# unilight/jatts

Measured on AMD Instinct MI355X. Metric: audio samples/sec (22.05 kHz) + RTF, FastSpeech2+HiFi-GAN, higher is better.
Workload: dtype f32 (emulated: 3 exact bf16 terms per operand, 7 MFMA products, f32 accumulate; attention / norms / duration predictor exact f32); 1 GPU; FastSpeech2(JSUT conformer 4+4, adim 384)+HiFi-GAN v1 22k, 64 utts x 128 phonemes x 6 frames per GPU; hop=256, parallelism=dp1 (utterance sharding, int16 PCM all-gather)

## Files before the change

### include/jatts_hip.h

```cpp
#ifndef JATTS_HIP_H_
#define JATTS_HIP_H_

#include <stdint.h>

#ifdef __cplusplus
extern "C" {
#endif

#define JATTS_ABI_VERSION 7

#define JATTS_F32 0
#define JATTS_F16 1
#define JATTS_F32S 2
#define JATTS_F32E 3
#define JATTS_F32E6 4

#define JATTS_ACT_NONE 0
#define JATTS_ACT_RELU 1
#define JATTS_ACT_TANH 2
#define JATTS_ACT_SWISH 3
#define JATTS_ACT_MISH 4
#define JATTS_ACT_SNAKEBETA 5

#define JATTS_PAD_ZERO 0
#define JATTS_PAD_REFLECT 1

#define JATTS_PRE_NONE 0
#define JATTS_PRE_LRELU 1

#define JATTS_OK 0
#define JATTS_ERR_ARG (-1)
#define JATTS_ERR_HIP (-2)
#define JATTS_ERR_UNSUPPORTED (-3)

int jatts_abi_version(void);
const char* jatts_last_error(void);
int jatts_device_info(char* buf, int buflen);

typedef struct jatts_ragged {
  const int32_t* cu_rows;
  int32_t n_seq;
  int32_t max_len;
  int32_t len_mul;
  int32_t total_rows;
  const int32_t* host_lens;
} jatts_ragged;

typedef struct jatts_conv_desc {
  jatts_ragged rg;
  int32_t dtype;
  int32_t n_in;
  const void* x[3];
  int32_t ldx;
  float in_scale;
  int32_t pre_act;
  float pre_slope;
  const void* w;
  int32_t c_in;
  int32_t n_out;
  int32_t k_w;
  int32_t dil;
  int32_t pad;
  const float* bias;
  int32_t act;
  float alpha;
  const float* resid;
  int32_t ldr;
  void* y;
  int32_t ldy;
  int32_t y_is_f32;
  int32_t y_transposed;
  const int32_t* y_seq_col0;
  int32_t pad_mode;
  int32_t variant;
  const float* w_inv;
  const float* act_a;
  const float* act_b;
  int32_t n_split;
  int32_t ldy2;
  void* y2;
  const int32_t* y2_seq_col0;
  int32_t w_layout;
} jatts_conv_desc;

int jatts_conv1d(const jatts_conv_desc* d, void* stream);

int64_t jatts_conv_weight_index(int32_t n, int32_t tap, int32_t c, int32_t n_pad, int32_t c_in);

typedef struct jatts_resunit_desc {
  jatts_ragged rg;
  int32_t dtype;
  int32_t channels;
  int32_t k_w;
  int32_t dil;
  float slope;
  const void* x;
  void* y;
  const void* w1;
  const float* b1;
  const void* w2;
  const float* b2;
  const void* add0;
  const void* add1;
  float out_scale;
  const float* ws1;
  const float* ws2;
  int32_t w_layout;
  int32_t variant;
} jatts_resunit_desc;

int jatts_hifigan_resunit(const jatts_resunit_desc* d, void* stream);

int jatts_resunit_variant(const jatts_resunit_desc* d);

int jatts_resunit_single_conv(int32_t dtype, int32_t w_layout);

int64_t jatts_unit_weight_index_k32(int32_t n, int32_t tap, int32_t c, int32_t channels);

typedef struct jatts_resblock_desc {
  jatts_ragged rg;
  int32_t dtype;
  int32_t channels;
  int32_t k_w;
  int32_t n_units;
  int32_t dil[3];
  float slope;
  const void* x;
  void* y;
  const void* w1[3];
  const float* b1[3];
  const void* w2[3];
  const float* b2[3];
  const void* add0;
  const void* add1;
  float out_scale;
  const float* ws1[3];
  const float* ws2[3];
} jatts_resblock_desc;

int jatts_hifigan_resblock(const jatts_resblock_desc* d, void* stream);

int jatts_masked_loss(const jatts_ragged* rg, const float* a, int32_t lda, const float* b, int32_t ldb, int32_t dim,
                      const int32_t* valid_len, int32_t kind, float log_offset, double scale, float* out, double* workspace,
                      void* stream);
int jatts_conv1d_wgrad(const jatts_ragged* rg, const float* x, int32_t ldx, const float* dy, int32_t ldy, int32_t c_in,
                       int32_t n_out, int32_t k_w, int32_t dil, int32_t pad, float* dw, float* db, float* workspace, void* stream);
int jatts_pack_conv_weight(const float* w, int32_t n_out, int32_t c_in, int32_t k_w, int32_t c_mult, int32_t mode, int32_t dtype,
                           void* out, void* stream);
int jatts_pack_conv_weight_split(const float* w, int32_t n_out, int32_t c_in, int32_t k_w, int32_t c_mult, int32_t mode, void* out, float* inv,
                                 void* stream);
int jatts_pack_conv_weight_bf16x3(const float* w, int32_t n_out, int32_t c_in, int32_t k_w, int32_t c_mult, int32_t dgrad, void* out, void* stream);
int jatts_conv1d_wgrad_emul(const jatts_ragged* rg, const float* x, int32_t ldx, const float* dy, int32_t ldy, int32_t c_in, int32_t n_out, int32_t k_w,
                            int32_t dil, int32_t pad, int32_t dtype, float* dw, float* db, float* workspace, void* stream);
int jatts_col_sum(const float* x, int32_t ld, int64_t rows, int32_t dim, float* out, void* stream);

int jatts_layernorm_bwd(const float* x, int32_t ldx, const float* dy, int32_t lddy, const float* gamma, int64_t rows, int32_t dim,
                        float eps, float* dx, int32_t lddx, float* dgamma, float* dbeta, void* stream);
int jatts_act_fwd(int32_t mode, const float* x, float* y, int64_t n, void* stream);
int jatts_act_bwd(int32_t mode, const float* x, const float* dy, float* dx, int64_t n, void* stream);
int jatts_glu_fwd(const float* x, float* y, int64_t rows, int32_t dim, void* stream);
int jatts_glu_bwd(const float* x, const float* dy, float* dx, int64_t rows, int32_t dim, void* stream);
int jatts_dwconv(const jatts_ragged* rg, const float* x, const float* w, const float* bias, float* y, int32_t dim, int32_t k_w,
                 int32_t pad, int32_t flip, void* stream);
int jatts_dwconv_wgrad(const jatts_ragged* rg, const float* x, const float* dy, float* dw, int32_t dim, int32_t k_w, int32_t pad,
                       void* stream);
int jatts_col_stats(const float* x, const float* y2, int32_t ld, int64_t rows, int32_t dim, const float* shift, const float* mul,
                    int32_t mode, float* out0, float* out1, void* stream);
int jatts_bn_bwd_apply(const float* x, const float* dy, int64_t rows, int32_t dim, const float* mean, const float* rstd,
                       const float* gamma, const float* s_dy, const float* s_dyx, float* dx, void* stream);
int jatts_index_add_rows(const float* src, int32_t ld, const int64_t* idx, int64_t rows, int32_t dim, float scale, int64_t skip,
                         int64_t n_dst, float* dst, void* stream);
int jatts_lr_segment_sum(const jatts_ragged* rg, const int64_t* cum, const int32_t* cu_out, const float* dy, int32_t dim, float* dhs,
                         void* stream);
int jatts_shift_softmax_fwd(const float* ac, const float* bd, int32_t n_batch, int32_t n_heads, int32_t t_len, const int32_t* lens,
                            float scale, int32_t shift_mode, float* p, void* stream);
int jatts_shift_softmax_bwd(const float* p, const float* dp, int32_t n_batch, int32_t n_heads, int32_t t_len, float scale,
                            int32_t shift_mode, float* ds, float* dbd, void* stream);
int jatts_gate_bwd(const float* x, const float* dy, float* dx, int64_t rows, int32_t dim, void* stream);
int jatts_weight_norm_fwd(const float* v, const float* g, int32_t n_out, int32_t row_len, float* w, float* inv_norm, void* stream);
int jatts_weight_norm_bwd(const float* v, const float* g, const float* inv_norm, const float* dw, int32_t n_out, int32_t row_len,
                          float* dv, float* dg, void* stream);
int jatts_split_add(const float* o, const float* h, const float* skip, int64_t rows, int32_t dim, float* h_out, float* skip_out, void* stream);
int jatts_concat2(const float* a, const float* b, int64_t rows, int32_t dim, float* out, void* stream);
int jatts_outer_rows(const float* v, const float* w, const float* bias, int64_t rows, int32_t dim, int32_t accumulate, float* out,
                     void* stream);
int jatts_col_wsum(const float* x, int32_t ld, const float* v, int64_t rows, int32_t dim, float* out, void* stream);
int jatts_row_dot(const float* x, int32_t ld, const float* w, const float* bias, int64_t rows, int32_t dim, float* y, void* stream);
int jatts_masked_loss_bwd(const jatts_ragged* rg, const float* a, int32_t lda, const float* b, int32_t ldb, int32_t dim,
                          const int32_t* valid_len, int32_t kind, float log_offset, float scale, const float* upstream, float* da,
                          int32_t ldda, void* stream);
int jatts_groupnorm_fwd(const jatts_ragged* rg, const float* x, int32_t dim, int32_t groups, const float* gamma, const float* beta,
                        float eps, float* y, float* mean, float* rstd, void* stream);
int jatts_groupnorm_bwd(const jatts_ragged* rg, const float* x, const float* dy, int32_t dim, int32_t groups, const float* gamma,
                        const float* mean, const float* rstd, float* dx, float* dgamma, float* dbeta, void* stream);
int jatts_snakebeta_fwd(const float* x, float* y, int64_t rows, int32_t dim, const float* alpha, const float* beta, void* stream);
int jatts_snakebeta_bwd(const float* x, const float* dy, int64_t rows, int32_t dim, const float* alpha, const float* beta, float* dx,
                        float* dalpha, float* dbeta, void* stream);
int jatts_ctc_forward_sum(const float* log_p, int32_t n_batch, int32_t t_max, int32_t ld, const int32_t* ilens, const int32_t* olens,
                          int32_t max_ilen, float log_blank, float* workspace, float* nll, float* grad, float grad_scale, void* stream);
int jatts_seq_sum(const jatts_ragged* rg, const float* x, int32_t dim, float* out, void* stream);
int jatts_dropout(const float* x, float* y, int64_t n, float p, uint64_t seed, const uint64_t* seed_dev, void* stream);
int jatts_qkv_split(const float* qkv, const float* u, const float* v, int32_t n_batch, int32_t t_len, int32_t n_heads, int32_t d_k, float* qu,
                    float* qv, float* k, float* vv, void* stream);
int jatts_qkv_split_bwd(const float* dqu, const float* dqv, const float* dk, const float* dvv, int32_t n_batch, int32_t t_len, int32_t n_heads,
                        int32_t d_k, float* dqkv, float* du, float* dv, void* stream);
int jatts_act_dropout(int32_t mode, const float* x, const float* dy, float* out, int64_t n, float p, uint64_t seed, const uint64_t* seed_dev,
                      void* stream);
int jatts_dropout_add(const float* x, const float* resid, float* y, int64_t n, float p, float alpha, uint64_t seed, const uint64_t* seed_dev,
                      void* stream);
int jatts_gather_grads(const float* const* src, const int64_t* numel, const int64_t* dst_off, int32_t n, float* flat, int32_t accumulate,
                       void* stream);
int jatts_sumsq(const float* x, int64_t n, double* out, void* stream);
int jatts_adam_step(float* p, const float* g, float* m, float* v, int64_t n, double lr, double beta1, double beta2, double eps,
                    double weight_decay, int64_t step, const double* grad_sumsq, float max_norm, const float* hyper_dev, void* stream);

int jatts_debug_trace(void* buf, int64_t n_workgroups);

int jatts_mfma_probe(int32_t dtype, int32_t feed, const void* operands, int64_t operand_bytes, int32_t iters, int32_t workgroups,
                     uint64_t* clocks, float* sink, void* stream);
double jatts_mfma_probe_flops(int32_t dtype, int32_t iters, int32_t workgroups);

int jatts_bgemm(const float* a, int64_t sa_outer, int64_t sa_inner, int32_t lda, int32_t trans_a, const float* b, int64_t sb_outer,
                int64_t sb_inner, int32_t ldb, int32_t trans_b, float* c, int64_t sc_outer, int64_t sc_inner, int32_t ldc, int32_t n_outer,
                int32_t n_inner, int32_t m, int32_t n, int32_t k, float alpha, int32_t accumulate, void* stream);

int jatts_bgemm_emul(const float* a, int64_t sa_outer, int64_t sa_inner, int32_t lda, int32_t trans_a, const float* b, int64_t sb_outer,
                     int64_t sb_inner, int32_t ldb, int32_t trans_b, float* c, int64_t sc_outer, int64_t sc_inner, int32_t ldc, int32_t n_outer,
                     int32_t n_inner, int32_t m, int32_t n, int32_t k, float alpha, int32_t accumulate, int32_t arith, void* stream);

int jatts_set_workspace(void* buf, int64_t bytes);

int jatts_hifigan_output(const jatts_ragged* rg, int32_t dtype, const void* const* x, int32_t n_in,
                         float in_scale, float slope, int32_t c_in, int32_t k_w, const float* w,
                         float bias, float* y, void* stream);

typedef struct jatts_relattn_desc {
  jatts_ragged rg;
  int32_t dtype;
  int32_t n_heads;
  int32_t d_k;
  const void* q;  int32_t ldq;
  const void* k;  int32_t ldk;
  const void* vt; int32_t ldvt;
  const void* g;  int32_t ldg;
  const float* ku;
  float scale;
  void* out; int32_t ldo;
  int32_t rel_mode;
  int32_t rel_center;
  const int32_t* vt_col0;
  const int32_t* kv_len;
} jatts_relattn_desc;

int jatts_relpos_attention(const jatts_relattn_desc* d, void* stream);

int jatts_rowdot(int32_t dtype, const void* x, int32_t ldx, int64_t rows, int32_t n_heads,
                 int32_t d_k, const float* vec, float* out, void* stream);

int jatts_embed_scale(const int64_t* ids, int64_t rows, const float* table, int32_t dim,
                      float scale, float* out, int64_t vocab, int64_t* n_bad, void* stream);

int jatts_layernorm(const void* x, int32_t in_dtype, int32_t ldx, void* y, int32_t out_dtype,
                    int32_t ldy, int64_t rows, int32_t dim, const float* gamma,
                    const float* beta, float eps, void* stream);

int jatts_affine_cast(const float* x, int32_t ldx, void* y, int32_t out_dtype, int32_t ldy,
                      int64_t rows, int32_t dim, const float* scale, const float* shift,
                      void* stream);
int jatts_affine_slice(const float* x, int32_t ldx, void* y, int32_t out_dtype, int32_t ldy,
                      int64_t rows, int32_t dim, const float* scale, const float* shift,
                      void* stream);

int jatts_glu_dwconv_bn_swish(const jatts_ragged* rg, int32_t dtype, const void* x, void* y,
                              int32_t channels, int32_t k_w, const float* w_dw,
                              const float* bn_scale, const float* bn_shift, void* stream);

int jatts_predictor_head(int32_t dtype, const void* x, int32_t ldx, int64_t rows, int32_t dim,
                         const float* w, float b, float* v_out, int64_t* dur_out, float offset,
                         void* stream);

int jatts_variance_embed_add(const jatts_ragged* rg, float* hs, int32_t dim, const float* p,
                             const float* wp, const float* bp, int32_t kp, const float* e,
                             const float* we, const float* be, int32_t ke, void* stream);

int jatts_gated_tanh_sigmoid(const jatts_ragged* rg, int32_t dtype, const void* x, const float* gseq,
                             void* y, int32_t channels, void* stream);

int jatts_groupnorm_mish(const jatts_ragged* rg, const void* x, int32_t in_dtype, void* y, int32_t out_dtype,
                         int32_t channels, int32_t groups, const float* gamma, const float* beta, float eps,
                         const float* addvec, float* workspace, void* stream);

int jatts_snakebeta(int32_t dtype, const void* x, void* y, int64_t rows, int32_t channels, const float* alpha,
                    const float* inv_beta, void* stream);

int jatts_l2_normalize(const float* x, int32_t ldx, void* y, int32_t out_dtype, int32_t ldy, int64_t rows,
                       int32_t dim, float eps, void* stream);

int jatts_gaussian_sample(const float* stats, const float* noise, float* z, int64_t rows, int32_t channels,
                          float noise_scale, void* stream);

int jatts_flip_channels(const float* x, float* y, int64_t rows, int32_t channels, void* stream);

int jatts_add_seq_vector(const jatts_ragged* rg, float* hs, int32_t dim, const float* vec,
                         void* stream);

int jatts_frame_signal(const jatts_ragged* rg_frames, const int32_t* cu_samples, const float* x, const float* window,
                       int32_t n_fft, int32_t hop, float* out, int32_t ldo, void* stream);
int jatts_power_spectrum(const float* x, int32_t ldx, int32_t n_bins, int64_t rows, float* out, int32_t ldo, void* stream);
int jatts_fbank_post(const jatts_ragged* rg, const float* p, int32_t ldp, int32_t n_mels, float amin, float top_db,
                     float* out, int32_t ldo, void* stream);
int jatts_seq_mean_std(const jatts_ragged* rg, const float* x, int32_t ldx, int32_t dim, const float* logits, int32_t ldl,
                       float* mean, float* stdv, int32_t ldm, float eps, void* stream);
int jatts_seq_affine_act(const jatts_ragged* rg, const float* x, int32_t ldx, int32_t dim, const float* seq_vec, int32_t pre_act,
                         const float* scale, const float* shift, int32_t post_act, void* y, int32_t out_dtype, int32_t ldy,
                         void* stream);
int jatts_se_scale_add(const jatts_ragged* rg, const float* x, int32_t dim, const float* s, const float* resid, float* y, int32_t ldy,
                       void* stream);

int jatts_stft_mag(const jatts_ragged* rg_frames, const int32_t* cu_samples, const int32_t* host_samples, const float* x,
                   const float* table, int32_t n_fft, int32_t hop, float* mag, int32_t ldo, float* pow_sum, void* stream);
int jatts_logmel_post(const float* mel, int32_t ldm, int32_t n_mels, int64_t rows, float eps, int32_t log_base, float* out,
                      int32_t ldo, void* stream);
int jatts_energy_frames(const float* pow_sum, int64_t rows, float* e, void* stream);
int jatts_energy_adjust(const jatts_ragged* rg_in, const jatts_ragged* rg_out, const float* e, float* out, void* stream);
int jatts_token_average(const jatts_ragged* rg_tokens, const jatts_ragged* rg_frames, const int32_t* cum, const float* e, float* out,
                        void* stream);

int jatts_resample(int32_t n_seq, const int32_t* cu_in, const int32_t* cu_out, const int32_t* host_in, const float* x,
                   const float* table, int32_t up, int32_t down, int32_t half_len, int32_t table_rows, float* y, void* stream);
int jatts_wave_gain_peak(int32_t n_seq, const int32_t* cu, float* y, float gain, float* peak, void* stream);

int jatts_acf_from_mag(const jatts_ragged* rg_frames, const float* mag, int32_t ldm, const float* table, int32_t K, int32_t Lp,
                       float* r, void* stream);
int jatts_pitch_pick(const jatts_ragged* rg_frames, const float* r, int32_t ldr, const float* peak, int32_t peak_stride, int32_t lo,
                     int32_t hi, float sr, float f0min, float sum_w2, float voicing_threshold, float silence_threshold,
                     float octave_cost, float* f0, int32_t* tau, void* stream);
int jatts_f0_continuous_log(const jatts_ragged* rg_frames, const float* f0, int32_t use_continuous, int32_t use_log, float* out,
                            void* stream);

#define JATTS_STATS_ROWS_PER_GROUP 1024
int32_t jatts_stats_rows_per_group(void);
int jatts_col_moments(const float* x, int32_t ld, int32_t dim, int64_t rows, double* state, double* ws, int64_t ws_doubles,
                      void* stream);
int jatts_col_moments_merge(double* state, const double* other, int32_t dim, void* stream);
int jatts_standardize(const float* x, int32_t ldx, int32_t dim, int64_t rows, const float* mean, const float* scale, float* y,
                      int32_t ldy, void* stream);

int jatts_lr_durations(const jatts_ragged* rg, const int64_t* d, float alpha, int32_t zero_rule,
                       int64_t* d_eff, int64_t* cum, int64_t* olens, void* stream);
int jatts_lr_gather(const jatts_ragged* rg_in, const int64_t* cum, const int32_t* cu_out,
                    int32_t max_out_len, const float* x, int32_t dim, float* out,
                    int64_t* frame_index, void* stream);

int jatts_zero_pad_rows(const jatts_ragged* rg, void* x, int32_t dtype, int32_t ld, int32_t dim, const int32_t* valid_len,
                        void* stream);
int jatts_cfm_mix(const jatts_ragged* rg, const float* x1, const float* z, const float* t, float sigma_min, int32_t dim,
                  float* y, float* u, void* stream);
int jatts_sq_err_sum(const float* a, const float* b, int64_t n, float scale, float* out, double* workspace, void* stream);

int jatts_gaussian_upsample(const jatts_ragged* rg_in, const int64_t* d, const int32_t* cu_out,
                            int32_t max_out_len, const float* hs, int32_t dim, float delta,
                            float* out, void* stream);

int jatts_gaussian_upsample_fwd(const float* hs, const float* ds, const int32_t* kv, const int32_t* kvo, int32_t B, int32_t Tm, int32_t To,
                                int32_t C, float delta, float* out, float* stat, void* stream);
int jatts_gaussian_upsample_bwd(const float* g, const float* ds, const float* stat, const int32_t* kv, const int32_t* kvo, int32_t B, int32_t Tm,
                                int32_t To, int32_t C, float delta, float* d_hs, void* stream);

int jatts_pcm16(const float* x, int64_t n, int16_t* y, void* stream);

int jatts_alignment_logp(const jatts_ragged* rg_feats, const int32_t* cu_text, int32_t max_text_len, const float* feats,
                         const float* text, int32_t adim, float* log_p, int32_t ld, void* stream);

int jatts_alignment_logp_bwd(const jatts_ragged* rg_feats, const int32_t* cu_text, int32_t max_text_len, const float* feats,
                             const float* text, int32_t adim, const float* log_p, int32_t ld, const float* dlog_p, int32_t ld_g,
                             float* w, float* d_feats, float* d_text, void* stream);

int jatts_mas_viterbi(const jatts_ragged* rg_feats, const int32_t* cu_text, const float* log_p, int32_t ld,
                      int32_t max_text_len, int64_t* path, int64_t* dur, double* score, void* stream);

#ifdef __cplusplus
}
#endif
#endif
```

### jatts_amd/_abi.py

```python
import ctypes as C
import os

_HERE = os.path.dirname(os.path.abspath(__file__))
LIB_PATH = os.environ.get("JATTS_HIP_LIB") or os.path.join(_HERE, "lib", "libjatts_hip.so")

F32, F16, F32S, F32E, F32E6 = 0, 1, 2, 3, 4
ABI_VERSION = 7
ACT_NONE, ACT_RELU, ACT_TANH, ACT_SWISH, ACT_MISH, ACT_SNAKEBETA = 0, 1, 2, 3, 4, 5
PRE_NONE, PRE_LRELU = 0, 1
PAD_ZERO, PAD_REFLECT = 0, 1
STATS_ROWS_PER_GROUP = 1024


class Ragged(C.Structure):
    _fields_ = [("cu_rows", C.c_void_p), ("n_seq", C.c_int32), ("max_len", C.c_int32),
                ("len_mul", C.c_int32), ("total_rows", C.c_int32), ("host_lens", C.c_void_p)]


class ConvDesc(C.Structure):
    _fields_ = [
        ("rg", Ragged), ("dtype", C.c_int32), ("n_in", C.c_int32), ("x", C.c_void_p * 3),
        ("ldx", C.c_int32), ("in_scale", C.c_float), ("pre_act", C.c_int32), ("pre_slope", C.c_float),
        ("w", C.c_void_p), ("c_in", C.c_int32), ("n_out", C.c_int32), ("k_w", C.c_int32),
        ("dil", C.c_int32), ("pad", C.c_int32), ("bias", C.c_void_p), ("act", C.c_int32),
        ("alpha", C.c_float), ("resid", C.c_void_p), ("ldr", C.c_int32), ("y", C.c_void_p),
        ("ldy", C.c_int32), ("y_is_f32", C.c_int32), ("y_transposed", C.c_int32), ("y_seq_col0", C.c_void_p),
        ("pad_mode", C.c_int32), ("variant", C.c_int32), ("w_inv", C.c_void_p), ("act_a", C.c_void_p), ("act_b", C.c_void_p),
        ("n_split", C.c_int32), ("ldy2", C.c_int32), ("y2", C.c_void_p), ("y2_seq_col0", C.c_void_p), ("w_layout", C.c_int32),
    ]


class ResUnitDesc(C.Structure):
    _fields_ = [
        ("rg", Ragged), ("dtype", C.c_int32), ("channels", C.c_int32), ("k_w", C.c_int32),
        ("dil", C.c_int32), ("slope", C.c_float), ("x", C.c_void_p), ("y", C.c_void_p),
        ("w1", C.c_void_p), ("b1", C.c_void_p), ("w2", C.c_void_p), ("b2", C.c_void_p),
        ("add0", C.c_void_p), ("add1", C.c_void_p), ("out_scale", C.c_float),
        ("ws1", C.c_void_p), ("ws2", C.c_void_p), ("w_layout", C.c_int32), ("variant", C.c_int32),
    ]


class ResBlockDesc(C.Structure):
    _fields_ = [
        ("rg", Ragged), ("dtype", C.c_int32), ("channels", C.c_int32), ("k_w", C.c_int32), ("n_units", C.c_int32),
        ("dil", C.c_int32 * 3), ("slope", C.c_float), ("x", C.c_void_p), ("y", C.c_void_p),
        ("w1", C.c_void_p * 3), ("b1", C.c_void_p * 3), ("w2", C.c_void_p * 3), ("b2", C.c_void_p * 3),
        ("add0", C.c_void_p), ("add1", C.c_void_p), ("out_scale", C.c_float),
        ("ws1", C.c_void_p * 3), ("ws2", C.c_void_p * 3),
    ]


class RelAttnDesc(C.Structure):
    _fields_ = [
        ("rg", Ragged), ("dtype", C.c_int32), ("n_heads", C.c_int32), ("d_k", C.c_int32),
        ("q", C.c_void_p), ("ldq", C.c_int32), ("k", C.c_void_p), ("ldk", C.c_int32),
        ("vt", C.c_void_p), ("ldvt", C.c_int32), ("g", C.c_void_p), ("ldg", C.c_int32),
        ("ku", C.c_void_p), ("scale", C.c_float), ("out", C.c_void_p), ("ldo", C.c_int32),
        ("rel_mode", C.c_int32), ("rel_center", C.c_int32), ("vt_col0", C.c_void_p), ("kv_len", C.c_void_p),
    ]


PROTOTYPES = {
    "jatts_abi_version": (C.c_int, []),
    "jatts_last_error": (C.c_char_p, []),
    "jatts_device_info": (C.c_int, [C.c_char_p, C.c_int]),
    "jatts_conv1d": (C.c_int, [C.POINTER(ConvDesc), C.c_void_p]),
    "jatts_conv_weight_index": (C.c_int64, [C.c_int32] * 5),
    "jatts_hifigan_resunit": (C.c_int, [C.POINTER(ResUnitDesc), C.c_void_p]),
    "jatts_resunit_variant": (C.c_int, [C.POINTER(ResUnitDesc)]),
    "jatts_resunit_single_conv": (C.c_int, [C.c_int32, C.c_int32]),
    "jatts_unit_weight_index_k32": (C.c_int64, [C.c_int32] * 4),
    "jatts_hifigan_resblock": (C.c_int, [C.POINTER(ResBlockDesc), C.c_void_p]),
    "jatts_debug_trace": (C.c_int, [C.c_void_p, C.c_int64]),
    "jatts_mfma_probe": (C.c_int, [C.c_int32, C.c_int32, C.c_void_p, C.c_int64, C.c_int32, C.c_int32, C.c_void_p, C.c_void_p, C.c_void_p]),
    "jatts_mfma_probe_flops": (C.c_double, [C.c_int32, C.c_int32, C.c_int32]),
    "jatts_set_workspace": (C.c_int, [C.c_void_p, C.c_int64]),
    "jatts_pack_conv_weight_split": (C.c_int, [C.c_void_p, C.c_int32, C.c_int32, C.c_int32, C.c_int32, C.c_int32, C.c_void_p, C.c_void_p, C.c_void_p]),
    "jatts_bgemm": (C.c_int, [C.c_void_p, C.c_int64, C.c_int64, C.c_int32, C.c_int32, C.c_void_p, C.c_int64, C.c_int64, C.c_int32, C.c_int32,
                              C.c_void_p, C.c_int64, C.c_int64, C.c_int32, C.c_int32, C.c_int32, C.c_int32, C.c_int32, C.c_int32, C.c_float,
                              C.c_int32, C.c_void_p]),
    "jatts_bgemm_emul": (C.c_int, [C.c_void_p, C.c_int64, C.c_int64, C.c_int32, C.c_int32, C.c_void_p, C.c_int64, C.c_int64, C.c_int32, C.c_int32,
                                   C.c_void_p, C.c_int64, C.c_int64, C.c_int32, C.c_int32, C.c_int32, C.c_int32, C.c_int32, C.c_int32, C.c_float,
                                   C.c_int32, C.c_int32, C.c_void_p]),
    "jatts_pcm16": (C.c_int, [C.c_void_p, C.c_int64, C.c_void_p, C.c_void_p]),
    "jatts_alignment_logp": (C.c_int, [C.POINTER(Ragged), C.c_void_p, C.c_int32, C.c_void_p, C.c_void_p, C.c_int32,
                                       C.c_void_p, C.c_int32, C.c_void_p]),
    "jatts_alignment_logp_bwd": (C.c_int, [C.POINTER(Ragged), C.c_void_p, C.c_int32, C.c_void_p, C.c_void_p, C.c_int32, C.c_void_p, C.c_int32,
                                           C.c_void_p, C.c_int32, C.c_void_p, C.c_void_p, C.c_void_p, C.c_void_p]),
    "jatts_mas_viterbi": (C.c_int, [C.POINTER(Ragged), C.c_void_p, C.c_void_p, C.c_int32, C.c_int32, C.c_void_p,
                                    C.c_void_p, C.c_void_p, C.c_void_p]),
    "jatts_hifigan_output": (C.c_int, [C.POINTER(Ragged), C.c_int32, C.POINTER(C.c_void_p), C.c_int32,
                                       C.c_float, C.c_float, C.c_int32, C.c_int32, C.c_void_p, C.c_float,
                                       C.c_void_p, C.c_void_p]),
    "jatts_relpos_attention": (C.c_int, [C.POINTER(RelAttnDesc), C.c_void_p]),
    "jatts_rowdot": (C.c_int, [C.c_int32, C.c_void_p, C.c_int32, C.c_int64, C.c_int32, C.c_int32,
                               C.c_void_p, C.c_void_p, C.c_void_p]),
    "jatts_embed_scale": (C.c_int, [C.c_void_p, C.c_int64, C.c_void_p, C.c_int32, C.c_float, C.c_void_p,
                                    C.c_int64, C.c_void_p, C.c_void_p]),
    "jatts_layernorm": (C.c_int, [C.c_void_p, C.c_int32, C.c_int32, C.c_void_p, C.c_int32, C.c_int32,
                                  C.c_int64, C.c_int32, C.c_void_p, C.c_void_p, C.c_float, C.c_void_p]),
    "jatts_affine_cast": (C.c_int, [C.c_void_p, C.c_int32, C.c_void_p, C.c_int32, C.c_int32, C.c_int64,
                                    C.c_int32, C.c_void_p, C.c_void_p, C.c_void_p]),
    "jatts_affine_slice": (C.c_int, [C.c_void_p, C.c_int32, C.c_void_p, C.c_int32, C.c_int32, C.c_int64,
                                     C.c_int32, C.c_void_p, C.c_void_p, C.c_void_p]),
    "jatts_glu_dwconv_bn_swish": (C.c_int, [C.POINTER(Ragged), C.c_int32, C.c_void_p, C.c_void_p, C.c_int32,
                                            C.c_int32, C.c_void_p, C.c_void_p, C.c_void_p, C.c_void_p]),
    "jatts_predictor_head": (C.c_int, [C.c_int32, C.c_void_p, C.c_int32, C.c_int64, C.c_int32, C.c_void_p,
                                       C.c_float, C.c_void_p, C.c_void_p, C.c_float, C.c_void_p]),
    "jatts_variance_embed_add": (C.c_int, [C.POINTER(Ragged), C.c_void_p, C.c_int32, C.c_void_p, C.c_void_p,
                                           C.c_void_p, C.c_int32, C.c_void_p, C.c_void_p, C.c_void_p,
                                           C.c_int32, C.c_void_p]),
    "jatts_gated_tanh_sigmoid": (C.c_int, [C.POINTER(Ragged), C.c_int32, C.c_void_p, C.c_void_p, C.c_void_p,
                                           C.c_int32, C.c_void_p]),
    "jatts_groupnorm_mish": (C.c_int, [C.POINTER(Ragged), C.c_void_p, C.c_int32, C.c_void_p, C.c_int32, C.c_int32,
                                       C.c_int32, C.c_void_p, C.c_void_p, C.c_float, C.c_void_p, C.c_void_p, C.c_void_p]),
    "jatts_snakebeta": (C.c_int, [C.c_int32, C.c_void_p, C.c_void_p, C.c_int64, C.c_int32, C.c_void_p, C.c_void_p,
                                  C.c_void_p]),
    "jatts_l2_normalize": (C.c_int, [C.c_void_p, C.c_int32, C.c_void_p, C.c_int32, C.c_int32, C.c_int64, C.c_int32,
                                     C.c_float, C.c_void_p]),
    "jatts_gaussian_sample": (C.c_int, [C.c_void_p, C.c_void_p, C.c_void_p, C.c_int64, C.c_int32, C.c_float,
                                        C.c_void_p]),
    "jatts_flip_channels": (C.c_int, [C.c_void_p, C.c_void_p, C.c_int64, C.c_int32, C.c_void_p]),
    "jatts_add_seq_vector": (C.c_int, [C.POINTER(Ragged), C.c_void_p, C.c_int32, C.c_void_p, C.c_void_p]),
    "jatts_lr_durations": (C.c_int, [C.POINTER(Ragged), C.c_void_p, C.c_float, C.c_int32, C.c_void_p,
                                     C.c_void_p, C.c_void_p, C.c_void_p]),
    "jatts_lr_gather": (C.c_int, [C.POINTER(Ragged), C.c_void_p, C.c_void_p, C.c_int32, C.c_void_p,
                                  C.c_int32, C.c_void_p, C.c_void_p, C.c_void_p]),
    "jatts_frame_signal": (C.c_int, [C.POINTER(Ragged), C.c_void_p, C.c_void_p, C.c_void_p, C.c_int32, C.c_int32, C.c_void_p,
                                     C.c_int32, C.c_void_p]),
    "jatts_power_spectrum": (C.c_int, [C.c_void_p, C.c_int32, C.c_int32, C.c_int64, C.c_void_p, C.c_int32, C.c_void_p]),
    "jatts_fbank_post": (C.c_int, [C.POINTER(Ragged), C.c_void_p, C.c_int32, C.c_int32, C.c_float, C.c_float, C.c_void_p,
                                   C.c_int32, C.c_void_p]),
    "jatts_stft_mag": (C.c_int, [C.POINTER(Ragged), C.c_void_p, C.c_void_p, C.c_void_p, C.c_void_p, C.c_int32, C.c_int32, C.c_void_p,
                                 C.c_int32, C.c_void_p, C.c_void_p]),
    "jatts_logmel_post": (C.c_int, [C.c_void_p, C.c_int32, C.c_int32, C.c_int64, C.c_float, C.c_int32, C.c_void_p, C.c_int32, C.c_void_p]),
    "jatts_energy_frames": (C.c_int, [C.c_void_p, C.c_int64, C.c_void_p, C.c_void_p]),
    "jatts_energy_adjust": (C.c_int, [C.POINTER(Ragged), C.POINTER(Ragged), C.c_void_p, C.c_void_p, C.c_void_p]),
    "jatts_token_average": (C.c_int, [C.POINTER(Ragged), C.POINTER(Ragged), C.c_void_p, C.c_void_p, C.c_void_p, C.c_void_p]),
    "jatts_resample": (C.c_int, [C.c_int32, C.c_void_p, C.c_void_p, C.c_void_p, C.c_void_p, C.c_void_p, C.c_int32, C.c_int32, C.c_int32,
                                 C.c_int32, C.c_void_p, C.c_void_p]),
    "jatts_wave_gain_peak": (C.c_int, [C.c_int32, C.c_void_p, C.c_void_p, C.c_float, C.c_void_p, C.c_void_p]),
    "jatts_acf_from_mag": (C.c_int, [C.POINTER(Ragged), C.c_void_p, C.c_int32, C.c_void_p, C.c_int32, C.c_int32, C.c_void_p, C.c_void_p]),
    "jatts_pitch_pick": (C.c_int, [C.POINTER(Ragged), C.c_void_p, C.c_int32, C.c_void_p, C.c_int32, C.c_int32, C.c_int32, C.c_float,
                                   C.c_float, C.c_float, C.c_float, C.c_float, C.c_float, C.c_void_p, C.c_void_p, C.c_void_p]),
    "jatts_f0_continuous_log": (C.c_int, [C.POINTER(Ragged), C.c_void_p, C.c_int32, C.c_int32, C.c_void_p, C.c_void_p]),
    "jatts_stats_rows_per_group": (C.c_int32, []),
    "jatts_col_moments": (C.c_int, [C.c_void_p, C.c_int32, C.c_int32, C.c_int64, C.c_void_p, C.c_void_p, C.c_int64, C.c_void_p]),
    "jatts_col_moments_merge": (C.c_int, [C.c_void_p, C.c_void_p, C.c_int32, C.c_void_p]),
    "jatts_standardize": (C.c_int, [C.c_void_p, C.c_int32, C.c_int32, C.c_int64, C.c_void_p, C.c_void_p, C.c_void_p, C.c_int32, C.c_void_p]),
    "jatts_seq_mean_std": (C.c_int, [C.POINTER(Ragged), C.c_void_p, C.c_int32, C.c_int32, C.c_void_p, C.c_int32, C.c_void_p,
                                     C.c_void_p, C.c_int32, C.c_float, C.c_void_p]),
    "jatts_seq_affine_act": (C.c_int, [C.POINTER(Ragged), C.c_void_p, C.c_int32, C.c_int32, C.c_void_p, C.c_int32, C.c_void_p,
                                       C.c_void_p, C.c_int32, C.c_void_p, C.c_int32, C.c_int32, C.c_void_p]),
    "jatts_se_scale_add": (C.c_int, [C.POINTER(Ragged), C.c_void_p, C.c_int32, C.c_void_p, C.c_void_p, C.c_void_p, C.c_int32,
                                     C.c_void_p]),
    "jatts_masked_loss": (C.c_int, [C.POINTER(Ragged), C.c_void_p, C.c_int32, C.c_void_p, C.c_int32, C.c_int32, C.c_void_p,
                                    C.c_int32, C.c_float, C.c_double, C.c_void_p, C.c_void_p, C.c_void_p]),
    "jatts_conv1d_wgrad": (C.c_int, [C.POINTER(Ragged), C.c_void_p, C.c_int32, C.c_void_p, C.c_int32, C.c_int32, C.c_int32,
                                     C.c_int32, C.c_int32, C.c_int32, C.c_void_p, C.c_void_p, C.c_void_p, C.c_void_p]),
    "jatts_pack_conv_weight": (C.c_int, [C.c_void_p, C.c_int32, C.c_int32, C.c_int32, C.c_int32, C.c_int32, C.c_int32, C.c_void_p, C.c_void_p]),
    "jatts_pack_conv_weight_bf16x3": (C.c_int, [C.c_void_p, C.c_int32, C.c_int32, C.c_int32, C.c_int32, C.c_int32, C.c_void_p, C.c_void_p]),
    "jatts_conv1d_wgrad_emul": (C.c_int, [C.POINTER(Ragged), C.c_void_p, C.c_int32, C.c_void_p, C.c_int32, C.c_int32, C.c_int32,
                                          C.c_int32, C.c_int32, C.c_int32, C.c_int32, C.c_void_p, C.c_void_p, C.c_void_p, C.c_void_p]),
    "jatts_col_sum": (C.c_int, [C.c_void_p, C.c_int32, C.c_int64, C.c_int32, C.c_void_p, C.c_void_p]),
    "jatts_layernorm_bwd": (C.c_int, [C.c_void_p, C.c_int32, C.c_void_p, C.c_int32, C.c_void_p, C.c_int64, C.c_int32, C.c_float, C.c_void_p, C.c_int32, C.c_void_p, C.c_void_p, C.c_void_p]),
    "jatts_act_fwd": (C.c_int, [C.c_int32, C.c_void_p, C.c_void_p, C.c_int64, C.c_void_p]),
    "jatts_act_bwd": (C.c_int, [C.c_int32, C.c_void_p, C.c_void_p, C.c_void_p, C.c_int64, C.c_void_p]),
    "jatts_glu_fwd": (C.c_int, [C.c_void_p, C.c_void_p, C.c_int64, C.c_int32, C.c_void_p]),
    "jatts_glu_bwd": (C.c_int, [C.c_void_p, C.c_void_p, C.c_void_p, C.c_int64, C.c_int32, C.c_void_p]),
    "jatts_dwconv": (C.c_int, [C.POINTER(Ragged), C.c_void_p, C.c_void_p, C.c_void_p, C.c_void_p, C.c_int32, C.c_int32, C.c_int32, C.c_int32, C.c_void_p]),
    "jatts_dwconv_wgrad": (C.c_int, [C.POINTER(Ragged), C.c_void_p, C.c_void_p, C.c_void_p, C.c_int32, C.c_int32, C.c_int32, C.c_void_p]),
    "jatts_col_stats": (C.c_int, [C.c_void_p, C.c_void_p, C.c_int32, C.c_int64, C.c_int32, C.c_void_p, C.c_void_p, C.c_int32, C.c_void_p, C.c_void_p, C.c_void_p]),
    "jatts_bn_bwd_apply": (C.c_int, [C.c_void_p, C.c_void_p, C.c_int64, C.c_int32, C.c_void_p, C.c_void_p, C.c_void_p, C.c_void_p, C.c_void_p, C.c_void_p, C.c_void_p]),
    "jatts_index_add_rows": (C.c_int, [C.c_void_p, C.c_int32, C.c_void_p, C.c_int64, C.c_int32, C.c_float, C.c_int64, C.c_int64, C.c_void_p, C.c_void_p]),
    "jatts_lr_segment_sum": (C.c_int, [C.POINTER(Ragged), C.c_void_p, C.c_void_p, C.c_void_p, C.c_int32, C.c_void_p, C.c_void_p]),
    "jatts_shift_softmax_fwd": (C.c_int, [C.c_void_p, C.c_void_p, C.c_int32, C.c_int32, C.c_int32, C.c_void_p, C.c_float, C.c_int32, C.c_void_p, C.c_void_p]),
    "jatts_shift_softmax_bwd": (C.c_int, [C.c_void_p, C.c_void_p, C.c_int32, C.c_int32, C.c_int32, C.c_float, C.c_int32, C.c_void_p, C.c_void_p, C.c_void_p]),
    "jatts_gate_bwd": (C.c_int, [C.c_void_p, C.c_void_p, C.c_void_p, C.c_int64, C.c_int32, C.c_void_p]),
    "jatts_weight_norm_fwd": (C.c_int, [C.c_void_p, C.c_void_p, C.c_int32, C.c_int32, C.c_void_p, C.c_void_p, C.c_void_p]),
    "jatts_weight_norm_bwd": (C.c_int, [C.c_void_p, C.c_void_p, C.c_void_p, C.c_void_p, C.c_int32, C.c_int32, C.c_void_p, C.c_void_p, C.c_void_p]),
    "jatts_split_add": (C.c_int, [C.c_void_p, C.c_void_p, C.c_void_p, C.c_int64, C.c_int32, C.c_void_p, C.c_void_p, C.c_void_p]),
    "jatts_concat2": (C.c_int, [C.c_void_p, C.c_void_p, C.c_int64, C.c_int32, C.c_void_p, C.c_void_p]),
    "jatts_outer_rows": (C.c_int, [C.c_void_p, C.c_void_p, C.c_void_p, C.c_int64, C.c_int32, C.c_int32, C.c_void_p, C.c_void_p]),
    "jatts_col_wsum": (C.c_int, [C.c_void_p, C.c_int32, C.c_void_p, C.c_int64, C.c_int32, C.c_void_p, C.c_void_p]),
    "jatts_row_dot": (C.c_int, [C.c_void_p, C.c_int32, C.c_void_p, C.c_void_p, C.c_int64, C.c_int32, C.c_void_p, C.c_void_p]),
    "jatts_masked_loss_bwd": (C.c_int, [C.POINTER(Ragged), C.c_void_p, C.c_int32, C.c_void_p, C.c_int32, C.c_int32, C.c_void_p, C.c_int32, C.c_float, C.c_float, C.c_void_p, C.c_void_p, C.c_int32, C.c_void_p]),
    "jatts_groupnorm_fwd": (C.c_int, [C.POINTER(Ragged), C.c_void_p, C.c_int32, C.c_int32, C.c_void_p, C.c_void_p, C.c_float, C.c_void_p, C.c_void_p, C.c_void_p, C.c_void_p]),
    "jatts_groupnorm_bwd": (C.c_int, [C.POINTER(Ragged), C.c_void_p, C.c_void_p, C.c_int32, C.c_int32, C.c_void_p, C.c_void_p, C.c_void_p, C.c_void_p, C.c_void_p, C.c_void_p, C.c_void_p]),
    "jatts_snakebeta_fwd": (C.c_int, [C.c_void_p, C.c_void_p, C.c_int64, C.c_int32, C.c_void_p, C.c_void_p, C.c_void_p]),
    "jatts_snakebeta_bwd": (C.c_int, [C.c_void_p, C.c_void_p, C.c_int64, C.c_int32, C.c_void_p, C.c_void_p, C.c_void_p, C.c_void_p, C.c_void_p, C.c_void_p]),
    "jatts_ctc_forward_sum": (C.c_int, [C.c_void_p, C.c_int32, C.c_int32, C.c_int32, C.c_void_p, C.c_void_p, C.c_int32, C.c_float, C.c_void_p, C.c_void_p, C.c_void_p, C.c_float, C.c_void_p]),
    "jatts_seq_sum": (C.c_int, [C.POINTER(Ragged), C.c_void_p, C.c_int32, C.c_void_p, C.c_void_p]),
    "jatts_dropout": (C.c_int, [C.c_void_p, C.c_void_p, C.c_int64, C.c_float, C.c_uint64, C.c_void_p, C.c_void_p]),
    "jatts_qkv_split": (C.c_int, [C.c_void_p, C.c_void_p, C.c_void_p, C.c_int32, C.c_int32, C.c_int32, C.c_int32, C.c_void_p, C.c_void_p, C.c_void_p, C.c_void_p, C.c_void_p]),
    "jatts_qkv_split_bwd": (C.c_int, [C.c_void_p, C.c_void_p, C.c_void_p, C.c_void_p, C.c_int32, C.c_int32, C.c_int32, C.c_int32, C.c_void_p, C.c_void_p, C.c_void_p, C.c_void_p]),
    "jatts_act_dropout": (C.c_int, [C.c_int32, C.c_void_p, C.c_void_p, C.c_void_p, C.c_int64, C.c_float, C.c_uint64, C.c_void_p, C.c_void_p]),
    "jatts_dropout_add": (C.c_int, [C.c_void_p, C.c_void_p, C.c_void_p, C.c_int64, C.c_float, C.c_float, C.c_uint64, C.c_void_p, C.c_void_p]),
    "jatts_sumsq": (C.c_int, [C.c_void_p, C.c_int64, C.c_void_p, C.c_void_p]),
    "jatts_gather_grads": (C.c_int, [C.c_void_p, C.c_void_p, C.c_void_p, C.c_int32, C.c_void_p, C.c_int32, C.c_void_p]),
    "jatts_adam_step": (C.c_int, [C.c_void_p, C.c_void_p, C.c_void_p, C.c_void_p, C.c_int64, C.c_double, C.c_double, C.c_double, C.c_double, C.c_double, C.c_int64, C.c_void_p, C.c_float, C.c_void_p, C.c_void_p]),
    "jatts_zero_pad_rows": (C.c_int, [C.POINTER(Ragged), C.c_void_p, C.c_int32, C.c_int32, C.c_int32, C.c_void_p, C.c_void_p]),
    "jatts_cfm_mix": (C.c_int, [C.POINTER(Ragged), C.c_void_p, C.c_void_p, C.c_void_p, C.c_float, C.c_int32, C.c_void_p,
                                C.c_void_p, C.c_void_p]),
    "jatts_sq_err_sum": (C.c_int, [C.c_void_p, C.c_void_p, C.c_int64, C.c_float, C.c_void_p, C.c_void_p, C.c_void_p]),
    "jatts_gaussian_upsample": (C.c_int, [C.POINTER(Ragged), C.c_void_p, C.c_void_p, C.c_int32, C.c_void_p,
                                          C.c_int32, C.c_float, C.c_void_p, C.c_void_p]),
    "jatts_gaussian_upsample_fwd": (C.c_int, [C.c_void_p, C.c_void_p, C.c_void_p, C.c_void_p, C.c_int32, C.c_int32, C.c_int32, C.c_int32, C.c_float,
                                              C.c_void_p, C.c_void_p, C.c_void_p]),
    "jatts_gaussian_upsample_bwd": (C.c_int, [C.c_void_p, C.c_void_p, C.c_void_p, C.c_void_p, C.c_void_p, C.c_int32, C.c_int32, C.c_int32, C.c_int32,
                                              C.c_float, C.c_void_p, C.c_void_p]),
}

_lib = None


class JattsHipError(RuntimeError):
    pass


def load():
    global _lib
    if _lib is not None:
        return _lib
    if not os.path.exists(LIB_PATH):
        raise JattsHipError(
            f"{LIB_PATH} not found: build it with `python -c 'import __graft_entry__ as g; g.build()'` "
            "or `make -C jatts_amd/csrc`.  jatts_amd has no CPU fallback."
        )
    lib = C.CDLL(LIB_PATH)
    for name, (res, args) in PROTOTYPES.items():
        fn = getattr(lib, name)
        fn.restype, fn.argtypes = res, args
    if lib.jatts_abi_version() != ABI_VERSION:
        raise JattsHipError(f"libjatts_hip.so ABI version {lib.jatts_abi_version()} != {ABI_VERSION} (include/jatts_hip.h): rebuild with __graft_entry__.build()")
    if lib.jatts_stats_rows_per_group() != STATS_ROWS_PER_GROUP:
        raise JattsHipError(f"libjatts_hip.so sums statistics in groups of {lib.jatts_stats_rows_per_group()} rows, _abi.py says {STATS_ROWS_PER_GROUP}: rebuild")
    _lib = lib
    return lib


def check(rc, what=""):
    if rc != 0:
        msg = load().jatts_last_error().decode(errors="replace")
        raise JattsHipError(f"{what} failed (rc={rc}): {msg}")
```

### jatts_amd/csrc/conv1d_direct.h

```cpp
#pragma once
#include "conv1d_impl.h"
#include "unit_frame.h"

namespace {

typedef unsigned u32x4_t __attribute__((ext_vector_type(4)));

template <int NF, int NT>
__device__ __forceinline__ void apply_act_alpha(f32x16 (&acc)[NF][NT], int act, float alpha) {
#define JATTS_ACT_LOOP(A)                                      \
  _Pragma("unroll") for (int f = 0; f < NF; ++f)               \
  _Pragma("unroll") for (int t = 0; t < NT; ++t)               \
  _Pragma("unroll") for (int r = 0; r < 16; ++r) acc[f][t][r] = act_c<A>(acc[f][t][r]) * alpha;
  switch (act) {
    case JATTS_ACT_RELU: JATTS_ACT_LOOP(JATTS_ACT_RELU) break;
    case JATTS_ACT_TANH: JATTS_ACT_LOOP(JATTS_ACT_TANH) break;
    case JATTS_ACT_SWISH: JATTS_ACT_LOOP(JATTS_ACT_SWISH) break;
    case JATTS_ACT_MISH: JATTS_ACT_LOOP(JATTS_ACT_MISH) break;
    default:
      if (alpha != 1.f) { JATTS_ACT_LOOP(JATTS_ACT_NONE) }
      break;
  }
#undef JATTS_ACT_LOOP
}

template <int NF, int NT, int WN, int WT, int D, int DIAG = 0, bool PRE = false, bool SNAKE = false>
__global__ __launch_bounds__(WN* WT * 64, (D <= 2 ? 3 : 2)) void conv1d_direct_kernel(jatts_conv_desc d, unsigned long long* trace, unsigned trace_cap, XcdOrder xo) {
  int bx, by, bz;
  if (!xo.decode(blockIdx.x, bx, by, bz, d.rg, WT * NT * 32)) return;
  JATTS_TRACE_BEGIN(trace, trace_cap, blockIdx.x);
  constexpr int BT = WT * NT * 32;
  const int b = by;
  const int row_b = d.rg.cu_rows[b];
  const int L = (d.rg.cu_rows[b + 1] - row_b) * d.rg.len_mul;
  const int t0 = bx * BT;
  if (t0 >= L) return;
  const int64_t seq_row0 = (int64_t)row_b * d.rg.len_mul;
  const int lane = threadIdx.x & 63, wave = threadIdx.x >> 6;
  const int wn = wave / WT, wt = wave % WT;
  const int KC16 = d.c_in >> 4;
  const int n_pad = (d.n_out + 31) & ~31;
  const int NFR = n_pad >> 5;
  const int nf0 = (bz * WN + wn) * NF;
  const int col0 = wt * NT * 32;
  const int g = lane >> 5;
  conv_second_output(d, bz * WN * NF * 32);

  f32x16 acc[NF][NT];
  {
    const f32x16 zero = {0.f, 0.f, 0.f, 0.f, 0.f, 0.f, 0.f, 0.f, 0.f, 0.f, 0.f, 0.f, 0.f, 0.f, 0.f, 0.f};
#pragma unroll
    for (int f = 0; f < NF; ++f) {
      const int n = (nf0 + f) * 32 + (lane & 31);
      const float bv = (d.bias && g == 0 && n < d.n_out) ? d.bias[n] : 0.f;
#pragma unroll
      for (int t = 0; t < NT; ++t) acc[f][t] = __builtin_amdgcn_mfma_f32_32x32x2f32(bv, 1.f, zero, 0, 0, 0);
    }
  }

  const __amdgpu_buffer_rsrc_t rw = __builtin_amdgcn_make_buffer_rsrc((void*)d.w, 0, (unsigned)((size_t)d.k_w * KC16 * NFR * 2048), 0x00020000);
  const __amdgpu_buffer_rsrc_t rx = __builtin_amdgcn_make_buffer_rsrc((void*)((const float*)d.x[0] + seq_row0 * (int64_t)d.ldx), 0,
                                                                    (unsigned)(((int64_t)(L - 1) * d.ldx + d.c_in) * 4), 0x00020000);
  unsigned vw[NF], vx[NT];
#pragma unroll
  for (int f = 0; f < NF; ++f) vw[f] = (unsigned)(lane * 32 + (nf0 + f < NFR ? nf0 + f : NFR - 1) * 2048);
#pragma unroll
  for (int t = 0; t < NT; ++t) vx[t] = (unsigned)(((t0 + col0 + t * 32 + (lane & 31) - d.pad) * d.ldx + 8 * g) * 4);
  const unsigned tap_stride = (unsigned)(d.dil * d.ldx * 4);
  int p_kc = 0, p_tap = 0;
  const int last_kc = KC16 - 1, last_tap = d.k_w - 1;
  auto ldb8 = [](const __amdgpu_buffer_rsrc_t& r, unsigned voff, unsigned soff) {
    const f32x4 lo = __builtin_bit_cast(f32x4, __builtin_amdgcn_raw_buffer_load_b128(r, voff, soff, 0));
    const f32x4 hi = __builtin_bit_cast(f32x4, __builtin_amdgcn_raw_buffer_load_b128(r, voff + 16, soff, 0));
    return f32x8{lo[0], lo[1], lo[2], lo[3], hi[0], hi[1], hi[2], hi[3]};
  };
  auto issue = [&](f32x8(&a)[NF], f32x8(&bq)[NT]) {
    const unsigned sw = (unsigned)((p_tap * KC16 + p_kc) * NFR) << 11;
#pragma unroll
    for (int f = 0; f < NF; ++f) a[f] = ldb8(rw, vw[f], sw);
    const unsigned shift = (unsigned)p_tap * tap_stride, sx = (unsigned)p_kc << 6;
#pragma unroll
    for (int t = 0; t < NT; ++t) bq[t] = ldb8(rx, vx[t] + shift, sx);
    ++p_tap;
    if (p_tap > last_tap) { p_tap = 0; ++p_kc; }
    if (p_kc > last_kc) { p_kc = last_kc; p_tap = last_tap; }
  };
  f32x8 ra[D][NF], rb[D][NT];
#pragma unroll
  for (int j = 0; j < D; ++j) issue(ra[j], rb[j]);
  __builtin_amdgcn_sched_barrier(0);
  const int n_steps = KC16 * d.k_w;
  JATTS_STAMP(2);
  for (int s0 = 0; s0 < n_steps; s0 += D) {
#pragma unroll
    for (int j = 0; j < D; ++j) {
      if (PRE) {
#pragma unroll
        for (int t = 0; t < NT; ++t)
#pragma unroll
          for (int e = 0; e < 8; ++e) rb[j][t][e] = fmaxf(rb[j][t][e], rb[j][t][e] * d.pre_slope);
      }
#pragma unroll
      for (int f = 0; f < NF; ++f)
#pragma unroll
        for (int t = 0; t < NT; ++t) mma32(ra[j][f], rb[j][t], acc[f][t]);
      if (DIAG == 0) issue(ra[j], rb[j]);
      __builtin_amdgcn_sched_barrier(0);
    }
  }
  JATTS_STAMP(3);

  const bool rowmajor = !d.y_transposed && (d.n_out & 7) == 0 && (reinterpret_cast<uintptr_t>(d.y) & 15) == 0 && (d.ldy & 3) == 0 &&
                        (!d.resid || ((d.ldr & 3) == 0 && (reinterpret_cast<uintptr_t>(d.resid) & 15) == 0));
  if constexpr (SNAKE) snake_acc<NF, NT>(acc, d.act_a, d.act_b, nf0, d.n_out, lane);
  if (rowmajor) {
    apply_act_alpha<NF, NT>(acc, d.act, d.alpha);
    const __amdgpu_buffer_rsrc_t ry = __builtin_amdgcn_make_buffer_rsrc((void*)((float*)d.y + seq_row0 * (int64_t)d.ldy), 0,
                                                                      (unsigned)(((int64_t)(L - 1) * d.ldy + d.n_out) * 4), 0x00020000);
    const __amdgpu_buffer_rsrc_t rr = __builtin_amdgcn_make_buffer_rsrc((void*)(d.resid ? d.resid + seq_row0 * (int64_t)d.ldr : (const float*)d.y), 0,
                                                                      (unsigned)(((int64_t)(L - 1) * d.ldr + d.n_out) * 4), 0x00020000);
    const int nf0s = __builtin_amdgcn_readfirstlane(nf0);
#pragma unroll
    for (int t = 0; t < NT; ++t) {
      const int row = t0 + col0 + t * 32 + (lane & 31);
      const unsigned vy = (unsigned)((row * d.ldy + 4 * g) * 4), vr = (unsigned)((row * d.ldr + 4 * g) * 4);
#pragma unroll
      for (int f = 0; f < NF; ++f) {
        const int nb = (nf0s + f) * 32;
        if (nb >= d.n_out) continue;
#pragma unroll
        for (int q = 0; q < 4; ++q) {
          if (nb + 8 * q >= d.n_out) continue;
          f32x4 v = {acc[f][t][4 * q], acc[f][t][4 * q + 1], acc[f][t][4 * q + 2], acc[f][t][4 * q + 3]};
          const unsigned so = (unsigned)(nb + 8 * q) * 4;
          if (d.resid) v += __builtin_bit_cast(f32x4, __builtin_amdgcn_raw_buffer_load_b128(rr, vr, so, 0));
          __builtin_amdgcn_raw_buffer_store_b128(__builtin_bit_cast(u32x4_t, v), ry, vy, so, 0);
        }
      }
    }
  } else {
    switch (d.act) {
      case JATTS_ACT_RELU: conv_epilogue<float, JATTS_ACT_RELU, NF, NT>(d, acc, t0, col0, nf0, lane, L, seq_row0, b); break;
      case JATTS_ACT_TANH: conv_epilogue<float, JATTS_ACT_TANH, NF, NT>(d, acc, t0, col0, nf0, lane, L, seq_row0, b); break;
      case JATTS_ACT_SWISH: conv_epilogue<float, JATTS_ACT_SWISH, NF, NT>(d, acc, t0, col0, nf0, lane, L, seq_row0, b); break;
      case JATTS_ACT_MISH: conv_epilogue<float, JATTS_ACT_MISH, NF, NT>(d, acc, t0, col0, nf0, lane, L, seq_row0, b); break;
      default: conv_epilogue<float, JATTS_ACT_NONE, NF, NT>(d, acc, t0, col0, nf0, lane, L, seq_row0, b); break;
    }
  }
  JATTS_STAMP(4);
  JATTS_TRACE_END();
}

inline bool conv_direct_ok(const jatts_conv_desc& d) {
  const int64_t maxL = (int64_t)d.rg.max_len * d.rg.len_mul;
  const int64_t n_pad = (d.n_out + 31) & ~31;
  const int64_t ld = d.ldx > d.ldy ? (d.ldx > d.ldr ? d.ldx : d.ldr) : (d.ldy > d.ldr ? d.ldy : d.ldr);
  return d.n_in == 1 && d.in_scale == 1.f && (d.pre_act == JATTS_PRE_NONE || (d.pre_act == JATTS_PRE_LRELU && d.pre_slope >= 0.f && d.pre_slope <= 1.f)) &&
         d.pad_mode == JATTS_PAD_ZERO && (d.ldx & 3) == 0 &&
         (reinterpret_cast<uintptr_t>(d.x[0]) & 15) == 0 && (reinterpret_cast<uintptr_t>(d.w) & 15) == 0 &&
         (maxL + 256 + (int64_t)d.k_w * d.dil) * ld * 4 < (int64_t)1 << 31 && (int64_t)d.k_w * d.c_in * n_pad * 4 < (int64_t)1 << 31;
}

template <int NF, int NT, int WN, int WT, int D, int DIAG = 0, bool PRE = false, bool SNAKE = false>
int launch_conv_direct(const jatts_conv_desc& d, hipStream_t s) {
  constexpr int BT = WT * NT * 32, BN = WN * NF * 32;
  const int64_t maxL = (int64_t)d.rg.max_len * d.rg.len_mul;
  XcdOrder xo;
  const int64_t total = xo.plan((int)((maxL + BT - 1) / BT), d.rg.n_seq, (d.n_out + BN - 1) / BN, (int64_t)BN * d.c_in * d.k_w * 4, ragged_tiles_1d(d.rg, BT));
  if (total >= (int64_t)1 << 31) return jatts_set_error_msg(JATTS_ERR_UNSUPPORTED, "conv1d: launch too large");
  hipLaunchKernelGGL((conv1d_direct_kernel<NF, NT, WN, WT, D, DIAG, PRE, SNAKE>), dim3((unsigned)total), dim3(WN * WT * 64), 0, s, d, jatts_g_trace,
                     jatts_g_trace_cap, xo);
  JATTS_CHECK_LAUNCH();
  return JATTS_OK;
}

}
```

### jatts_amd/csrc/conv1d_emul.hip

```cpp
#include "conv1d_emul16.h"

template <typename T>
static int conv1d_emul(const jatts_conv_desc& d, hipStream_t s) {
  constexpr bool TWO = sizeof(typename Acc32<T>::type) > sizeof(f32x16);
  if (d.n_in > 1)
    return launch_conv_emul<T, 2, 2, 2, 2, 3, 32, 1>(d, s);
  if (d.n_out <= 64) return launch_conv_emul<T, 2, 1, 1, 4, 1, 32, 2>(d, s);
  const int64_t maxL = (int64_t)d.rg.max_len * d.rg.len_mul;
  const int64_t wgs128 = ((maxL + 127) / 128) * d.rg.n_seq * ((d.n_out + 127) / 128);
  const bool small_k1 = d.k_w == 1 && wgs128 <= 768;
  if (TWO && d.k_w > 1 && wgs128 <= 128 && (d.k_w - 1) * d.dil <= 32) return launch_conv_emul<T, 1, 2, 4, 1, 1, 64, 2, 32, 4>(d, s);
  if (d.k_w == 1 && (TWO || small_k1)) return launch_conv_emul<T, 1, 2, 4, 1, 1, 64, 2, 32, 4>(d, s);
  if constexpr (TWO) return launch_conv_emul<T, 1, 2, 4, 2, 1, 64, 1, 32, 4>(d, s);
  else return launch_conv_emul<T, 2, 2, 2, 2, 1, 32, 2>(d, s);
}

template <typename T>
static int conv1d_emul16(const jatts_conv_desc& d, hipStream_t s) {
  const int variant = d.variant;
  if (d.n_in > 1) return launch_conv_emul16<T, 4, 4, 2, 2, 3, 64, 1>(d, s);
  if (d.n_out <= 64) return launch_conv_emul16<T, 2, 2, 2, 2, 1, 64, 2>(d, s);
  const int64_t maxL = (int64_t)d.rg.max_len * d.rg.len_mul;
  const int64_t t64 = ((maxL + 63) / 64) * d.rg.n_seq;
  const int64_t wgs128 = ((maxL + 127) / 128) * d.rg.n_seq * ((d.n_out + 127) / 128);
  const bool ok384 = d.n_split % 384 == 0;
  if (ok384 && (variant == 6 || (variant == 0 && d.n_out % 384 == 0 && t64 * (d.n_out / 384) >= 256))) return launch_conv_emul16<T, 3, 4, 8, 1, 1, 64, 1, 32, 1>(d, s);
  if (variant == 3 || (variant == 0 && d.n_out % 256 == 0 && t64 * (d.n_out / 256) >= 256)) return launch_conv_emul16<T, 2, 4, 8, 1, 1, 64, 1>(d, s);
  if (variant == 9 || (variant == 0 && t64 * ((d.n_out + 127) / 128) <= 256)) return launch_conv_emul16<T, 2, 2, 4, 1, 1, 64, 2>(d, s);
  if (variant == 1 || (variant == 0 && (d.k_w == 1 || wgs128 <= 128))) return launch_conv_emul16<T, 2, 4, 4, 1, 1, 64, 2>(d, s);
  return launch_conv_emul16<T, 2, 4, 4, 2, 1, 64, 1>(d, s);
}

int jatts_conv1d_emul(const jatts_conv_desc& d, hipStream_t s) {
  if (d.w_layout == 1) return d.dtype == JATTS_F32E6 ? conv1d_emul16<bf3f>(d, s) : conv1d_emul16<bf3>(d, s);
  return d.dtype == JATTS_F32E6 ? conv1d_emul<bf3f>(d, s) : conv1d_emul<bf3>(d, s);
}
```

### jatts_amd/csrc/conv1d_emul16.h

```cpp
#pragma once
#include "conv1d_emul.h"
#include "unit_frame.h"
#include "resunit_emul16_impl.h"

#ifndef JATTS_CEMUL_ANTIPHASE
#define JATTS_CEMUL_ANTIPHASE 1
#endif
#ifndef JATTS_CEMUL_TRACE
#define JATTS_CEMUL_TRACE 0
#endif
#if JATTS_CEMUL_TRACE
#define JATTS_CEMUL_TRACE_PARAMS , unsigned long long* trace, unsigned trace_cap
#else
#define JATTS_CEMUL_TRACE_PARAMS
#endif

namespace {

template <typename T, int NF, int D>
struct WRing16 {
  typedef typename Elem<T>::vec8 V8;
  V8 r[D][NF];
  const T* wbase;
  int nfo[NF];
  int KC32, NFR16, k_w, kc_per, n_chunks;
  int p_chunk, p_tap, p_kk;

  __device__ __forceinline__ void init(const T* w, int KC32_, int NFR16_, int nf0, int k_w_, int kc_per_, int n_chunks_, int lane) {
    wbase = w + (size_t)lane * 8;
    KC32 = KC32_; NFR16 = NFR16_; k_w = k_w_; kc_per = kc_per_; n_chunks = n_chunks_;
#pragma unroll
    for (int f = 0; f < NF; ++f) nfo[f] = (nf0 + f < NFR16 ? nf0 + f : NFR16 - 1) * 512;
    p_chunk = p_tap = p_kk = 0;
#pragma unroll
    for (int j = 0; j < D; ++j) {
#pragma unroll
      for (int f = 0; f < NF; ++f) fetch_frag(j, f);
      advance();
    }
  }
  __device__ __forceinline__ const T* pos() const { return wbase + ((size_t)(p_tap * KC32 + p_chunk * kc_per + p_kk) * NFR16) * 512; }
  __device__ __forceinline__ void fetch_frag(int j, int f) { r[j][f] = Vec8IO<T>::ldg(pos() + nfo[f]); }
  __device__ __forceinline__ void advance() {
    const int nk = p_kk + 1;
    const bool wk = nk == kc_per;
    p_kk = wk ? 0 : nk;
    const int nt = p_tap + (wk ? 1 : 0);
    const bool wt = nt == k_w;
    p_tap = wt ? 0 : nt;
    const int nc = p_chunk + (wt ? 1 : 0);
    const bool end = nc == n_chunks;
    p_chunk = end ? n_chunks - 1 : nc;
    p_tap = end ? k_w - 1 : p_tap;
    p_kk = end ? kc_per - 1 : p_kk;
  }
};

template <typename T, int NF, int NT, int D>
__device__ __forceinline__ void conv_stage16(typename Acc16<T>::type (&acc)[NF][NT], WRing16<T, NF, D>& ring, int kc_per, int k_w, int dil, const char* act,
                                             int pitch, int col0, int lane) {
  typedef typename Elem<T>::vec8 V8;
  static_assert(NT % 2 == 0, "column fragments come in pairs");
  const int n_it = k_w * kc_per;
  const char* bbase = act + (size_t)(col0 + (lane & 15)) * pitch + (size_t)(lane >> 4) * 48;
  const int last_tap = k_w - 1;
  int bp_tap = 0, bp_kk = 0;
  auto next_b = [&]() {
    const int nk = bp_kk + 1;
    const bool wrap = nk == kc_per;
    const bool end = wrap && bp_tap == last_tap;
    bp_kk = end ? bp_kk : (wrap ? 0 : nk);
    bp_tap = end ? bp_tap : bp_tap + (wrap ? 1 : 0);
    return bbase + (size_t)(bp_tap * dil) * pitch + (size_t)(bp_kk * 4) * 48;
  };
  V8 rb[NT];
#pragma unroll
  for (int t = 0; t < NT; ++t) rb[t] = Vec8IO<T>::lds(bbase + (size_t)(t * 16) * pitch);
  __builtin_amdgcn_sched_barrier(0);
  for (int it0 = 0; it0 < n_it; it0 += D) {
#pragma unroll
    for (int j = 0; j < D; ++j) {
      const char* pb = next_b();
#pragma unroll
      for (int f = 0; f < NF; ++f) {
#pragma unroll
        for (int tp = 0; tp < NT; tp += 2) {
          pair16<T, NF, NT>(acc, ring.r[j][f], rb, f, tp);
          if (f == NF - 1 && !(JATTS_CEMUL_DIAG & 16)) {
            rb[tp] = Vec8IO<T>::lds(pb + (size_t)(tp * 16) * pitch);
            rb[tp + 1] = Vec8IO<T>::lds(pb + (size_t)((tp + 1) * 16) * pitch);
          }
          __builtin_amdgcn_sched_barrier(0);
        }
        if (!(JATTS_CEMUL_DIAG & 8)) ring.fetch_frag(j, f);
        __builtin_amdgcn_sched_barrier(0);
      }
      ring.advance();
    }
  }
}

template <int NF, int NT>
__device__ __forceinline__ void snake_acc16(f32x4 (&acc)[NF][NT], const float* a, const float* b, int nf0, int n_out, int lane) {
#pragma unroll
  for (int f = 0; f < NF; ++f) {
    const int n0 = min((nf0 + f) * 16 + 4 * (lane >> 4), n_out - 4);
    const f32x4 a4 = *reinterpret_cast<const f32x4*>(a + n0), b4 = *reinterpret_cast<const f32x4*>(b + n0);
#pragma unroll
    for (int t = 0; t < NT; ++t)
#pragma unroll
      for (int e = 0; e < 4; ++e) {
        const float v = acc[f][t][e];
        acc[f][t][e] = fmaf(b4[e], sin2_f(v * a4[e]), v);
      }
    __builtin_amdgcn_sched_barrier(0);
  }
}

template <int ACT, int NF, int NT>
__device__ __forceinline__ void conv_epilogue16(const jatts_conv_desc& d, f32x4 (&acc)[NF][NT], int t0, int col0, int nf0, int lane, int L, int64_t seq_row0,
                                                int seq) {
  const bool vec_r = d.resid && (d.ldr & 3) == 0, vec_y = (d.ldy & 3) == 0 && !d.y_transposed;
#pragma unroll
  for (int t = 0; t < NT; ++t) {
    const int pos = t0 + col0 + t * 16 + (lane & 15);
    if (pos >= L) continue;
    const int64_t row = seq_row0 + pos;
    const int64_t trow = d.y_seq_col0 ? (int64_t)d.y_seq_col0[seq] * d.rg.len_mul + pos : row;
#pragma unroll
    for (int f = 0; f < NF; ++f) {
      const int n0 = (nf0 + f) * 16 + 4 * (lane >> 4);
      if (n0 >= d.n_out) continue;
      const bool full = n0 + 3 < d.n_out;
      f32x4 rq = {0.f, 0.f, 0.f, 0.f};
      if (full && vec_r) rq = *reinterpret_cast<const f32x4*>(d.resid + row * d.ldr + n0);
      f32x4 v;
#pragma unroll
      for (int e = 0; e < 4; ++e) v[e] = act_c<ACT>(acc[f][t][e]) * d.alpha + rq[e];
      if (full && vec_y && (vec_r || !d.resid)) {
        *reinterpret_cast<f32x4*>((float*)d.y + row * d.ldy + n0) = v;
      } else {
#pragma unroll
        for (int e = 0; e < 4; ++e) {
          const int n = n0 + e;
          if (n >= d.n_out) break;
          float s = v[e];
          if (!full) s = act_c<ACT>(acc[f][t][e]) * d.alpha;
          if (d.resid && !(full && vec_r)) s += d.resid[row * d.ldr + n];
          const int64_t o = d.y_transposed ? (int64_t)n * d.ldy + trow : row * d.ldy + n;
          ((float*)d.y)[o] = s;
        }
      }
      __builtin_amdgcn_sched_barrier(0);
    }
  }
}

template <int ACT, int NF, int NT, int BN>
__device__ __forceinline__ void conv_epilogue_lds16(const jatts_conv_desc& d, f32x4 (&acc)[NF][NT], char* smem, int t0, int col0, int nf_local0, int n_base,
                                                    int lane, int L, int64_t seq_row0, int BT) {
  constexpr int opitch = BN * 4 + 16;
#pragma unroll
  for (int t = 0; t < NT; ++t) {
    const int col = col0 + t * 16 + (lane & 15);
#pragma unroll
    for (int f = 0; f < NF; ++f) {
      const int nl = (nf_local0 + f) * 16 + 4 * (lane >> 4);
      if (n_base + nl >= d.n_out) continue;
      f32x4 o;
#pragma unroll
      for (int e = 0; e < 4; ++e) o[e] = act_c<ACT>(acc[f][t][e]) * d.alpha;
      *reinterpret_cast<f32x4*>(smem + (size_t)col * opitch + (size_t)nl * 4) = o;
    }
  }
  __syncthreads();
  const int vrows = min(BT, L - t0);
  const int upr = min(BN, d.n_out - n_base) / 8;
  const int total = vrows * upr;
  float* yg = (float*)d.y + (seq_row0 + t0) * (int64_t)d.ldy + n_base;
  const float* rg = d.resid ? d.resid + (seq_row0 + t0) * (int64_t)d.ldr + n_base : nullptr;
  for (int u = threadIdx.x; u < total; u += blockDim.x) {
    const int r = u / upr, cu = u - r * upr;
    const char* src = smem + (size_t)r * opitch + (size_t)cu * 32;
    float* dst = yg + (int64_t)r * d.ldy + cu * 8;
    f32x4 lo = *reinterpret_cast<const f32x4*>(src), hi = *reinterpret_cast<const f32x4*>(src + 16);
    if (rg) {
      const float* rp = rg + (int64_t)r * d.ldr + cu * 8;
      lo += *reinterpret_cast<const f32x4*>(rp);
      hi += *reinterpret_cast<const f32x4*>(rp + 4);
    }
    *reinterpret_cast<f32x4*>(dst) = lo;
    *reinterpret_cast<f32x4*>(dst + 4) = hi;
  }
}

template <typename T, int NF, int NT, int WN, int WT, int NIN, int KCHT, int OCC, int HALO = 32, int D = 2>
__global__ __launch_bounds__(WN* WT * 64, OCC) void conv1d_emul16_kernel(jatts_conv_desc d, int f32_tile, XcdOrder xo JATTS_CEMUL_TRACE_PARAMS) {
  extern __shared__ __attribute__((aligned(16))) char smem[];
  constexpr int BT = WT * NT * 16, NTHR = WN * WT * 64, BN = WN * NF * 16;
  int bx, b, bz;
  if (!xo.decode(blockIdx.x, bx, b, bz, d.rg, BT)) return;
#if JATTS_CEMUL_TRACE
  const bool tracing = trace != nullptr && blockIdx.x < trace_cap && threadIdx.x == 0;
  unsigned long long ph[7] = {0, 0, 0, 0, 0, 0, 0}, tq = __builtin_amdgcn_s_memtime();
  const unsigned long long t_begin = tq, rt_begin = __builtin_amdgcn_s_memrealtime();
#define JATTS_PH(i) do { const unsigned long long n_ = __builtin_amdgcn_s_memtime(); ph[i] += n_ - tq; tq = n_; } while (0)
#else
#define JATTS_PH(i) do {} while (0)
#endif
  const int row_b = d.rg.cu_rows[b];
  const int L = (d.rg.cu_rows[b + 1] - row_b) * d.rg.len_mul;
  const int t0 = bx * BT;
  if (t0 >= L) return;
  const int64_t seq_row0 = (int64_t)row_b * d.rg.len_mul;
  const int lane = threadIdx.x & 63, wave = threadIdx.x >> 6;
  const int wn = wave / WT, wt = wave % WT;
  constexpr int pitch = KCHT * 6 + 16;
  const int rows = BT + (d.k_w - 1) * d.dil;
  const int KC32 = d.c_in >> 5;
  const int n_pad = (d.n_out + 31) & ~31;
  const int NFR16 = n_pad >> 4;
  const int nf0 = (bz * WN + wn) * NF;
  const int col0 = wt * NT * 16;
  conv_second_output(d, bz * BN);

  const float* xin[3] = {(const float*)d.x[0], (const float*)d.x[1], (const float*)d.x[2]};
  const bool reflect = d.pad_mode == JATTS_PAD_REFLECT;
  typename Acc16<T>::type accx[NF][NT];
  {
    const int g4 = lane >> 4;
#pragma unroll
    for (int f = 0; f < NF; ++f) {
      const int n0 = (nf0 + f) * 16 + 4 * g4;
      f32x4 bq = {0.f, 0.f, 0.f, 0.f};
      if (d.bias) {
        if (n0 + 3 < d.n_out) bq = *reinterpret_cast<const f32x4*>(d.bias + n0);
        else {
#pragma unroll
          for (int e = 0; e < 4; ++e)
            if (n0 + e < d.n_out) bq[e] = d.bias[n0 + e];
        }
      }
#pragma unroll
      for (int t = 0; t < NT; ++t)
#pragma unroll
        for (int e = 0; e < 4; ++e) acc16_set(accx[f][t], e, bq[e]);
    }
  }

  constexpr int UPRC = KCHT / 8;
  constexpr int MAXU = ((BT + HALO) * UPRC + NTHR - 1) / NTHR;
  static_assert((KCHT / 32) % D == 0 || D % (KCHT / 32) == 0, "ring depth and steps per chunk and tap");
  WRing16<T, NF, D> ring;
  const int n_chunks = d.c_in / KCHT;
  ring.init((const T*)d.w, KC32, NFR16, nf0, d.k_w, KCHT / 32, n_chunks, lane);
  const size_t buf_bytes = (size_t)rows * pitch;
  StageRegs<float, MAXU, NIN> sr;
  int64_t soff[MAXU];
  bool sok[MAXU];
  {
    const int total = rows * UPRC;
#pragma unroll
    for (int j = 0; j < MAXU; ++j) {
      const int u = threadIdx.x + j * NTHR;
      const int r = u / UPRC, cu = u % UPRC;
      int pos = t0 - d.pad + r;
      if (reflect) pos = reflect_pos(pos, L);
      sok[j] = u < total && pos >= 0 && pos < L;
      soff[j] = (seq_row0 + (sok[j] ? pos : 0)) * (int64_t)d.ldx + cu * 8;
#pragma unroll
      for (int i = 0; i < NIN; ++i)
#pragma unroll
        for (int e = 0; e < 8; ++e) sr.v[i][j][e] = 0.f;
    }
  }
  auto issue = [&](int c0) {
#pragma unroll
    for (int j = 0; j < MAXU; ++j)
#pragma unroll
      for (int i = 0; i < NIN; ++i)
        if (i < d.n_in && sok[j]) sr.v[i][j] = Vec8IO<float>::ldg(xin[i] + soff[j] + c0);
  };
  auto commit = [&](int ci) {
    emul_commit<T, MAXU, NIN, UPRC, NTHR>(sr, smem + (size_t)(ci & 1) * buf_bytes, pitch, rows, d.n_in, d.in_scale, d.pre_act, d.pre_slope);
  };
  const bool early = JATTS_CEMUL_ANTIPHASE && WN * WT == 8 && OCC == 1 && wave >= 4;
  issue(0);
  commit(0);
  if (early && n_chunks > 1) issue(KCHT);
  __syncthreads();
  JATTS_PH(0);
  for (int ci = 0; ci < n_chunks; ++ci) {
    const bool more = ci + 1 < n_chunks;
    if (early) {
      if (more) commit(ci + 1);
      if (ci + 2 < n_chunks) issue((ci + 2) * KCHT);
    } else if (more && !(JATTS_CEMUL_DIAG & 2)) issue((ci + 1) * KCHT);
    JATTS_PH(1);
    conv_stage16<T, NF, NT, D>(accx, ring, KCHT / 32, d.k_w, d.dil, smem + (size_t)(ci & 1) * buf_bytes, pitch, col0, lane);
    JATTS_PH(2);
#if JATTS_CEMUL_TRACE
    asm volatile("s_waitcnt vmcnt(0)" ::: "memory");
    JATTS_PH(3);
#endif
    if (!early && more && !(JATTS_CEMUL_DIAG & 64)) commit(ci + 1);
    JATTS_PH(4);
    if (!(JATTS_CEMUL_DIAG & 4)) __syncthreads();
    JATTS_PH(5);
  }
  if (JATTS_CEMUL_DIAG & 4) __syncthreads();

  f32x4 acc[NF][NT];
#pragma unroll
  for (int f = 0; f < NF; ++f)
#pragma unroll
    for (int t = 0; t < NT; ++t) {
      acc16_finish(accx[f][t]);
      acc[f][t] = acc16_val(accx[f][t]);
    }
  if (d.act == JATTS_ACT_SNAKEBETA) snake_acc16<NF, NT>(acc, d.act_a, d.act_b, nf0, d.n_out, lane);
#if JATTS_CEMUL_TRACE
  auto trace_out = [&]() {
    JATTS_PH(6);
    if (!tracing) return;
    unsigned long long* o = trace + (size_t)blockIdx.x * 16;
    JATTS_TRACE_HWID(hwid, xcc);
    o[0] = ((unsigned long long)(xcc & 0xF) << 32) | hwid;
    for (int i = 0; i < 7; ++i) o[1 + i] = ph[i];
    o[8] = rt_begin; o[9] = __builtin_amdgcn_s_memrealtime(); o[10] = t_begin; o[11] = tq;
  };
#else
  auto trace_out = []() {};
#endif
  if (JATTS_CEMUL_DIAG & 32) {
    float s = 0.f;
#pragma unroll
    for (int f = 0; f < NF; ++f)
#pragma unroll
      for (int t = 0; t < NT; ++t) s += acc[f][t][0] + acc[f][t][1] + acc[f][t][2] + acc[f][t][3];
    if (s != 12345.678f) return;
  }
  {
    const int n_base = bz * BN;
    const bool rowmajor = !d.y_transposed && (d.n_out & 7) == 0 && (reinterpret_cast<uintptr_t>(d.y) & 15) == 0;
    if (rowmajor && f32_tile && (d.ldy & 3) == 0 && (!d.resid || ((d.ldr & 3) == 0 && (reinterpret_cast<uintptr_t>(d.resid) & 15) == 0))) {
      switch (d.act) {
        case JATTS_ACT_RELU: conv_epilogue_lds16<JATTS_ACT_RELU, NF, NT, BN>(d, acc, smem, t0, col0, wn * NF, n_base, lane, L, seq_row0, BT); break;
        case JATTS_ACT_TANH: conv_epilogue_lds16<JATTS_ACT_TANH, NF, NT, BN>(d, acc, smem, t0, col0, wn * NF, n_base, lane, L, seq_row0, BT); break;
        case JATTS_ACT_SWISH: conv_epilogue_lds16<JATTS_ACT_SWISH, NF, NT, BN>(d, acc, smem, t0, col0, wn * NF, n_base, lane, L, seq_row0, BT); break;
        case JATTS_ACT_MISH: conv_epilogue_lds16<JATTS_ACT_MISH, NF, NT, BN>(d, acc, smem, t0, col0, wn * NF, n_base, lane, L, seq_row0, BT); break;
        default: conv_epilogue_lds16<JATTS_ACT_NONE, NF, NT, BN>(d, acc, smem, t0, col0, wn * NF, n_base, lane, L, seq_row0, BT); break;
      }
      trace_out();
      return;
    }
  }
  switch (d.act) {
    case JATTS_ACT_RELU: conv_epilogue16<JATTS_ACT_RELU, NF, NT>(d, acc, t0, col0, nf0, lane, L, seq_row0, b); break;
    case JATTS_ACT_TANH: conv_epilogue16<JATTS_ACT_TANH, NF, NT>(d, acc, t0, col0, nf0, lane, L, seq_row0, b); break;
    case JATTS_ACT_SWISH: conv_epilogue16<JATTS_ACT_SWISH, NF, NT>(d, acc, t0, col0, nf0, lane, L, seq_row0, b); break;
    case JATTS_ACT_MISH: conv_epilogue16<JATTS_ACT_MISH, NF, NT>(d, acc, t0, col0, nf0, lane, L, seq_row0, b); break;
    default: conv_epilogue16<JATTS_ACT_NONE, NF, NT>(d, acc, t0, col0, nf0, lane, L, seq_row0, b); break;
  }
  trace_out();
}

template <typename T, int NF, int NT, int WN, int WT, int NIN, int KCHT, int OCC, int HALO = 32, int D = 2>
int launch_conv_emul16(const jatts_conv_desc& d, hipStream_t s) {
  constexpr int BT = WT * NT * 16, BN = WN * NF * 16;
  if ((d.k_w - 1) * d.dil > HALO) return jatts_set_error_msg(JATTS_ERR_UNSUPPORTED, "conv1d (emulated): halo beyond the staging registers");
  if (d.c_in % KCHT) return jatts_set_error_msg(JATTS_ERR_UNSUPPORTED, "conv1d (emulated): c_in must be a multiple of the chunk width");
  const int64_t maxL = (int64_t)d.rg.max_len * d.rg.len_mul;
  dim3 grid((unsigned)((maxL + BT - 1) / BT), (unsigned)d.rg.n_seq, (unsigned)((d.n_out + BN - 1) / BN));
  const size_t rows = (size_t)BT + (size_t)(d.k_w - 1) * d.dil;
  size_t lds = 2 * rows * (KCHT * 6 + 16);
  int f32_tile = 0;
  const bool direct_epi = d.resid == nullptr;
  if (!direct_epi && !d.y_transposed && (size_t)BT * (BN * 4 + 16) <= 159 * 1024) {
    f32_tile = 1;
    if (lds < (size_t)BT * (BN * 4 + 16)) lds = (size_t)BT * (BN * 4 + 16);
  }
  constexpr auto kern = conv1d_emul16_kernel<T, NF, NT, WN, WT, NIN, KCHT, OCC, HALO, D>;
  if (const int rc = unit_lds_ready<kern>(JATTS_SITE("conv1d (emulated): tile exceeds 160 KiB LDS"), lds)) return rc;
  XcdOrder xo;
  const int64_t total = xo.plan((int)grid.x, (int)grid.y, (int)grid.z, (int64_t)BN * d.c_in * d.k_w * 6, ragged_tiles_1d(d.rg, BT));
  if (total >= (int64_t)1 << 31) return jatts_set_error_msg(JATTS_ERR_UNSUPPORTED, "conv1d: launch too large");
#if JATTS_CEMUL_TRACE
  hipLaunchKernelGGL(kern, dim3((unsigned)total), dim3(WN * WT * 64), lds, s, d, f32_tile, xo, jatts_g_trace, jatts_g_trace_cap);
#else
  hipLaunchKernelGGL(kern, dim3((unsigned)total), dim3(WN * WT * 64), lds, s, d, f32_tile, xo);
#endif
  JATTS_CHECK_LAUNCH();
  return JATTS_OK;
}

}
```

### jatts_amd/csrc/conv1d_f32_direct.hip

```cpp
#include "conv1d_direct.h"

int jatts_conv1d_f32_direct(const jatts_conv_desc& d, int variant, hipStream_t s) {
  if (!conv_direct_ok(d)) return 1;
  const bool snake = d.act == JATTS_ACT_SNAKEBETA;
  if (snake && (d.n_out <= 64 || d.pre_act != JATTS_PRE_NONE || (variant != 0 && variant != 3 && variant != 5))) return 1;
  if (d.n_out <= 64) {
    if (variant != 0 && variant != 3) return 1;
    return d.pre_act != JATTS_PRE_NONE ? launch_conv_direct<2, 2, 1, 4, 2, 0, true>(d, s) : launch_conv_direct<2, 2, 1, 4, 2>(d, s);
  }
  if (variant == 0) {
    const int64_t maxL = (int64_t)d.rg.max_len * d.rg.len_mul;
    const int64_t t128 = (maxL + 127) / 128, t64 = (maxL + 63) / 64;
    const int64_t wgs = t128 * d.rg.n_seq * ((d.n_out + 127) / 128);
    variant = (wgs <= 512 || t64 * 64 * 23 <= t128 * 128 * 20) ? 5 : 3;
  }
  if (d.pre_act != JATTS_PRE_NONE) {
    if (variant == 5) return launch_conv_direct<2, 1, 2, 2, 2, 0, true>(d, s);
    return launch_conv_direct<2, 2, 2, 2, 2, 0, true>(d, s);
  }
  if (snake) return variant == 5 ? launch_conv_direct<2, 1, 2, 2, 2, 0, false, true>(d, s) : launch_conv_direct<2, 2, 2, 2, 2, 0, false, true>(d, s);
  switch (variant) {
    case 3: return launch_conv_direct<2, 2, 2, 2, 2>(d, s);
    case 4: return launch_conv_direct<2, 2, 2, 2, 4>(d, s);
    case 5: return launch_conv_direct<2, 1, 2, 2, 2>(d, s);
#ifdef JATTS_DIAG
    case 8: return launch_conv_direct<2, 2, 2, 2, 2, 1>(d, s);
#endif
    default: return 1;
  }
}
```

### jatts_amd/csrc/conv_api.hip

```cpp
#include <stdlib.h>

#include "common.h"

unsigned long long* jatts_g_trace = nullptr;
unsigned jatts_g_trace_cap = 0;

int jatts_conv1d_f16(const jatts_conv_desc& d, hipStream_t s);
int jatts_conv1d_f32(const jatts_conv_desc& d, hipStream_t s);
int jatts_conv1d_split(const jatts_conv_desc& d, hipStream_t s);
int jatts_conv1d_emul(const jatts_conv_desc& d, hipStream_t s);
int jatts_resunit_f16_narrow(const jatts_resunit_desc& d, hipStream_t s);
int jatts_resunit_f16_wide(const jatts_resunit_desc& d, hipStream_t s);
int jatts_resunit_f32(const jatts_resunit_desc& d, hipStream_t s);
int jatts_resunit_split(const jatts_resunit_desc& d, hipStream_t s);
int jatts_resunit_emul(const jatts_resunit_desc& d, hipStream_t s, int* pick);
int jatts_resunit1_f16(const jatts_resunit_desc& d, hipStream_t s);
int jatts_resunit1_f32(const jatts_resunit_desc& d, hipStream_t s);
int jatts_resunit1_emul(const jatts_resunit_desc& d, hipStream_t s);
int jatts_resblock_f16(const jatts_resblock_desc& d, hipStream_t s);
int jatts_resblock_f32(const jatts_resblock_desc& d, hipStream_t s);
int jatts_resblock_split(const jatts_resblock_desc& d, hipStream_t s);
int jatts_resblock_emul(const jatts_resblock_desc& d, hipStream_t s);

extern "C" int jatts_debug_trace(void* buf, int64_t n_workgroups) {
  jatts_g_trace = (unsigned long long*)buf;
  jatts_g_trace_cap = buf ? (unsigned)n_workgroups : 0u;
  return JATTS_OK;
}

extern "C" int64_t jatts_conv_weight_index(int32_t n, int32_t tap, int32_t c, int32_t n_pad, int32_t c_in) {
  const int64_t KC16 = c_in / 16, NFR = n_pad / 32;
  const int64_t kc = c / 16, nf = n / 32;
  const int64_t lane = 32 * ((c % 16) / 8) + (n % 32);
  return ((((int64_t)tap * KC16 + kc) * NFR + nf) * 64 + lane) * 8 + (c % 8);
}

extern "C" int64_t jatts_unit_weight_index_k32(int32_t n, int32_t tap, int32_t c, int32_t channels) {
  const int64_t KC32 = channels / 32, NFR16 = channels / 16;
  const int64_t kc = c / 32, nf = n / 16;
  const int64_t lane = 16 * ((c % 32) / 8) + (n % 16);
  return ((((int64_t)tap * KC32 + kc) * NFR16 + nf) * 64 + lane) * 8 + (c % 8);
}

extern "C" int jatts_conv1d(const jatts_conv_desc* d, void* stream) {
  if (!d || !d->x[0] || !d->w || !d->y || !d->rg.cu_rows) return jatts_set_error_msg(JATTS_ERR_ARG, "conv1d: null pointer");
  if (d->c_in <= 0 || d->c_in % 64) return jatts_set_error_msg(JATTS_ERR_ARG, "conv1d: c_in must be a positive multiple of 64");
  if (d->ldx % 8) return jatts_set_error_msg(JATTS_ERR_ARG, "conv1d: ldx must be a multiple of 8");
  if (d->n_in < 1 || d->n_in > 3 || d->k_w < 1 || d->dil < 1 || d->n_out < 1 || d->rg.n_seq < 1 || d->rg.len_mul < 1)
    return jatts_set_error_msg(JATTS_ERR_ARG, "conv1d: bad geometry");
  if (d->pad < 0 || (int64_t)d->pad > (int64_t)(d->k_w - 1) * d->dil)
    return jatts_set_error_msg(JATTS_ERR_ARG, "conv1d: pad must lie in [0, (k_w - 1) * dil]");
  if (d->act == JATTS_ACT_SNAKEBETA && (!d->act_a || !d->act_b || (d->n_out & 3) || ((uintptr_t)d->act_a & 15) || ((uintptr_t)d->act_b & 15)))
    return jatts_set_error_msg(JATTS_ERR_ARG, "conv1d: JATTS_ACT_SNAKEBETA needs 16-byte aligned act_a / act_b and n_out % 4 == 0");
  if (d->n_split != 0 && (d->n_split < 0 || d->n_split % 256 || d->n_split >= d->n_out || !d->y2 || d->y_transposed || d->resid || d->ldy2 <= 0))
    return jatts_set_error_msg(JATTS_ERR_ARG, "conv1d: n_split must be a multiple of 256 below n_out, with y2 / ldy2 set, y row-major and no residual");
  if (d->w_layout != 0 && d->dtype != JATTS_F32E && d->dtype != JATTS_F32E6) return jatts_set_error_msg(JATTS_ERR_ARG, "conv1d: w_layout = 1 goes with JATTS_F32E / JATTS_F32E6 only");
  if (d->rg.max_len <= 0) return JATTS_OK;
  hipStream_t s = (hipStream_t)stream;
  if (d->dtype == JATTS_F16) return jatts_conv1d_f16(*d, s);
  if (d->dtype == JATTS_F32) return jatts_conv1d_f32(*d, s);
  if (d->dtype == JATTS_F32S) {
    if (!d->w_inv) return jatts_set_error_msg(JATTS_ERR_ARG, "conv1d: JATTS_F32S needs w_inv");
    if (!d->y_is_f32) return jatts_set_error_msg(JATTS_ERR_ARG, "conv1d: JATTS_F32S writes f32 (y_is_f32 = 1)");
    return jatts_conv1d_split(*d, s);
  }
  if (d->dtype == JATTS_F32E || d->dtype == JATTS_F32E6) {
    if (!d->y_is_f32) return jatts_set_error_msg(JATTS_ERR_ARG, "conv1d: JATTS_F32E / JATTS_F32E6 write f32 (y_is_f32 = 1)");
    if (d->w_layout != 0 && d->w_layout != 1) return jatts_set_error_msg(JATTS_ERR_ARG, "conv1d: w_layout must be 0 or 1");
    return jatts_conv1d_emul(*d, s);
  }
  return jatts_set_error_msg(JATTS_ERR_ARG, "conv1d: unknown dtype");
}

static int resunit_check(const jatts_resunit_desc* d) {
  if (!d || !d->x || !d->y || !d->w1 || !d->b1 || !d->rg.cu_rows) return jatts_set_error_msg(JATTS_ERR_ARG, "resunit: null pointer");
  if (!d->w2) {
    if (d->b2 || d->ws2) return jatts_set_error_msg(JATTS_ERR_ARG, "resunit: w2 == NULL (single-conv unit) takes b2 == NULL and ws2 == NULL");
  } else if (!d->b2) {
    return jatts_set_error_msg(JATTS_ERR_ARG, "resunit: null pointer");
  }
  if (d->x == d->y) return jatts_set_error_msg(JATTS_ERR_ARG, "resunit: y must not alias x");
  if (d->k_w < 1 || !(d->k_w & 1) || d->dil < 1) return jatts_set_error_msg(JATTS_ERR_ARG, "resunit: odd k_w and dil>=1 required");
  if (!(d->slope >= 0.f && d->slope <= 1.f)) return jatts_set_error_msg(JATTS_ERR_ARG, "resunit: LeakyReLU slope must be in [0, 1]");
  return JATTS_OK;
}

extern "C" int jatts_resunit_single_conv(int32_t dtype, int32_t w_layout) {
  if (dtype == JATTS_F32 || dtype == JATTS_F16) return w_layout == 0;
  return (dtype == JATTS_F32E || dtype == JATTS_F32E6) && w_layout == 1;
}

static int resunit1_check(const jatts_resunit_desc* d) {
  if (d->dtype == JATTS_F32S)
    return jatts_set_error_msg(JATTS_ERR_UNSUPPORTED, "resunit: the single-conv unit (w2 == NULL) has no JATTS_F32S kernel (JATTS_F32 / JATTS_F16 / JATTS_F32E / JATTS_F32E6)");
  if (d->dtype == JATTS_F32E || d->dtype == JATTS_F32E6) {
    if (d->w_layout != 0 && d->w_layout != 1) return jatts_set_error_msg(JATTS_ERR_ARG, "resunit: w_layout must be 0 or 1");
    if (d->w_layout != 1)
      return jatts_set_error_msg(JATTS_ERR_UNSUPPORTED, "resunit: the emulated single-conv unit (w2 == NULL) takes w_layout = 1 weights only");
    return JATTS_OK;
  }
  if (d->w_layout != 0) return jatts_set_error_msg(JATTS_ERR_ARG, "resunit: w_layout = 1 goes with JATTS_F32E / JATTS_F32E6 only");
  if (d->dtype != JATTS_F16 && d->dtype != JATTS_F32) return jatts_set_error_msg(JATTS_ERR_UNSUPPORTED, "resunit: unsupported channels/dtype (use jatts_conv1d)");
  return JATTS_OK;
}

extern "C" int jatts_hifigan_resunit(const jatts_resunit_desc* d, void* stream) {
  if (const int rc = resunit_check(d)) return rc;
  hipStream_t s = (hipStream_t)stream;
  if (!d->w2) {
    if (const int rc = resunit1_check(d)) return rc;
    if (d->rg.max_len <= 0) return JATTS_OK;
    if (d->dtype == JATTS_F16) return jatts_resunit1_f16(*d, s);
    if (d->dtype == JATTS_F32) return jatts_resunit1_f32(*d, s);
    return jatts_resunit1_emul(*d, s);
  }
  if (d->rg.max_len <= 0) return JATTS_OK;
  if (d->dtype == JATTS_F16) return d->channels <= 64 ? jatts_resunit_f16_narrow(*d, s) : jatts_resunit_f16_wide(*d, s);
  if (d->dtype == JATTS_F32) return jatts_resunit_f32(*d, s);
  if (d->dtype == JATTS_F32S) {
    if (!d->ws1 || !d->ws2) return jatts_set_error_msg(JATTS_ERR_ARG, "resunit: JATTS_F32S needs ws1 / ws2");
    return jatts_resunit_split(*d, s);
  }
  if (d->dtype == JATTS_F32E || d->dtype == JATTS_F32E6) {
    if (d->w_layout != 0 && d->w_layout != 1) return jatts_set_error_msg(JATTS_ERR_ARG, "resunit: w_layout must be 0 or 1");
    return jatts_resunit_emul(*d, s, nullptr);
  }
  if (d->w_layout != 0) return jatts_set_error_msg(JATTS_ERR_ARG, "resunit: w_layout = 1 goes with JATTS_F32E / JATTS_F32E6 only");
  return jatts_set_error_msg(JATTS_ERR_UNSUPPORTED, "resunit: unsupported channels/dtype (use jatts_conv1d)");
}

extern "C" int jatts_resunit_variant(const jatts_resunit_desc* d) {
  if (const int rc = resunit_check(d)) return rc;
  int form = 1;
  if (!d->w2) {
    const int rc = resunit1_check(d);
    return rc ? rc : 1;
  }
  if (d->rg.max_len > 0 && (d->dtype == JATTS_F32E || d->dtype == JATTS_F32E6)) {
    if (d->w_layout != 0 && d->w_layout != 1) return jatts_set_error_msg(JATTS_ERR_ARG, "resunit: w_layout must be 0 or 1");
    if (const int rc = jatts_resunit_emul(*d, nullptr, &form)) return rc;
  }
  return form;
}

extern "C" int jatts_hifigan_resblock(const jatts_resblock_desc* d, void* stream) {
  if (!d || !d->x || !d->y || !d->rg.cu_rows) return jatts_set_error_msg(JATTS_ERR_ARG, "resblock: null pointer");
  if (d->n_units < 1 || d->n_units > 3) return jatts_set_error_msg(JATTS_ERR_ARG, "resblock: 1..3 units");
  for (int u = 0; u < d->n_units; ++u) {
    if (!d->w1[u] || !d->w2[u] || !d->b1[u] || !d->b2[u]) return jatts_set_error_msg(JATTS_ERR_ARG, "resblock: null weights");
    if (d->dil[u] < 1) return jatts_set_error_msg(JATTS_ERR_ARG, "resblock: dil >= 1 required");
  }
  if (d->x == d->y) return jatts_set_error_msg(JATTS_ERR_ARG, "resblock: y must not alias x");
  if (d->k_w < 1 || !(d->k_w & 1)) return jatts_set_error_msg(JATTS_ERR_ARG, "resblock: odd k_w required");
  if (!(d->slope >= 0.f && d->slope <= 1.f)) return jatts_set_error_msg(JATTS_ERR_ARG, "resblock: LeakyReLU slope must be in [0, 1]");
  if (d->dtype == JATTS_F32S) {
    for (int u = 0; u < d->n_units; ++u)
      if (!d->ws1[u] || !d->ws2[u]) return jatts_set_error_msg(JATTS_ERR_ARG, "resblock: JATTS_F32S needs ws1 / ws2");
    if (d->rg.max_len <= 0) return JATTS_OK;
    return jatts_resblock_split(*d, (hipStream_t)stream);
  }
  if (d->dtype == JATTS_F32E || d->dtype == JATTS_F32E6) {
    if (d->rg.max_len <= 0) return JATTS_OK;
    return jatts_resblock_emul(*d, (hipStream_t)stream);
  }
  if (d->dtype != JATTS_F16 && d->dtype != JATTS_F32) return jatts_set_error_msg(JATTS_ERR_ARG, "resblock: unknown dtype");
  if (d->rg.max_len <= 0) return JATTS_OK;
  return d->dtype == JATTS_F16 ? jatts_resblock_f16(*d, (hipStream_t)stream) : jatts_resblock_f32(*d, (hipStream_t)stream);
}
```

### jatts_amd/hip.py

```python
import collections
import contextlib
import ctypes as C

import torch

from . import _abi
from . import precision as _precision
from ._abi import ACT_MISH, ACT_NONE, ACT_RELU, ACT_SWISH, ACT_TANH, F16, F32, F32E, F32E6, F32S
from .precision import EMUL, PRECISIONS

_TORCH = {F32: torch.float32, F16: torch.float16, F32S: torch.float32, F32E: torch.float32, F32E6: torch.float32}


def torch_dtype(code):
    return _TORCH[code]


def code_of(t):
    if t.dtype == torch.float32:
        return F32
    if t.dtype == torch.float16:
        return F16
    raise TypeError(f"unsupported dtype {t.dtype}")

# ... 171 lines not shown
        raise _abi.JattsHipError("jatts_amd kernels need device tensors (no CPU fallback)")
    return t


_KEEP = [None]


def keep_begin():
    _KEEP[0] = []
    return _KEEP[0]


def keep_end():
    _KEEP[0] = None


def keep(t):
    if _KEEP[0] is not None and t is not None:
        _KEEP[0].append(t)
    return t


def h2d(values, dtype, device):
    dev = torch.device(device)
    if dev.type != "cuda":
        return torch.tensor(values, dtype=dtype, device=dev)
    key = None
    if isinstance(values, (list, tuple)) and len(values) <= 65536 and all(isinstance(v, (int, float, bool)) for v in values[:1] + values[-1:]):
        key = (tuple(values), dtype, dev.index if dev.index is not None else torch.cuda.current_device())
        hit = _H2D_CACHE.get(key)
        if hit is not None:
            _H2D_CACHE.move_to_end(key)
            if hit[2] != torch.cuda.current_stream().cuda_stream and not torch.cuda.is_current_stream_capturing() and not hit[1].query():
                torch.cuda.current_stream().wait_event(hit[1])
            return keep(hit[0])
    if torch.cuda.is_current_stream_capturing():
        raise _abi.JattsHipError("h2d of new values while a graph is being captured: run the step once outside the capture first")
    t = torch.tensor(values, dtype=dtype).pin_memory().to(dev, non_blocking=True)
    if key is not None:
        ev = torch.cuda.Event()
        ev.record()
        _H2D_CACHE[key] = (t, ev, torch.cuda.current_stream().cuda_stream)
        _H2D_BYTES[0] += t.numel() * t.element_size()
        while _H2D_BYTES[0] > _H2D_CACHE_MAX_BYTES and len(_H2D_CACHE) > 1:
            _, old = _H2D_CACHE.popitem(last=False)
            _H2D_BYTES[0] -= old[0].numel() * old[0].element_size()
    return keep(t)


_H2D_CACHE = collections.OrderedDict()
_H2D_BYTES = [0]
_H2D_CACHE_MAX_BYTES = 8 << 20
_GEOM_CACHE = {}
_GEOM_CACHE_MAX = 512


def exclusive_scan(lens):
    cu = [0]
    for v in lens:
        cu.append(cu[-1] + v)
    return cu


class RaggedBatch:

    def __init__(self, lens, device):
        self.lens = [int(v) for v in lens]
        self.cu_host = cu = exclusive_scan(self.lens)
        self.total = cu[-1]
        self.n_seq = len(self.lens)
        self.max_len = max(self.lens) if self.lens else 0
        self.device = device
        dev = torch.device(device)
        if dev.type != "cuda":
            self.cu = torch.tensor(cu, dtype=torch.int32, device=dev)
            return
        key = (tuple(self.lens), dev.index if dev.index is not None else torch.cuda.current_device())
        hit = _GEOM_CACHE.get(key)
        if hit is None:
            t = h2d(cu, torch.int32, dev)
            ev = torch.cuda.Event()
            ev.record()
            if len(_GEOM_CACHE) >= _GEOM_CACHE_MAX:
                _GEOM_CACHE.pop(next(iter(_GEOM_CACHE)))
            _GEOM_CACHE[key] = hit = (t, ev, torch.cuda.current_stream().cuda_stream)
        elif hit[2] != torch.cuda.current_stream().cuda_stream and not torch.cuda.is_current_stream_capturing() and not hit[1].query():
            torch.cuda.current_stream().wait_event(hit[1])
        self.cu = keep(hit[0])

    def struct(self, len_mul=1):
        if _RAGGED_1D and self.n_seq > 1 and min(self.lens) != self.max_len:
            if not hasattr(self, "_lens_c"):
                self._lens_c = (C.c_int32 * self.n_seq)(*self.lens)
            return _abi.Ragged(self.cu.data_ptr(), self.n_seq, self.max_len, len_mul, self.total, C.addressof(self._lens_c))
        return _abi.Ragged(self.cu.data_ptr(), self.n_seq, self.max_len, len_mul, 0, None)

    def vt_layout(self):
        if not hasattr(self, "_vt"):
            col, c = [], 0
            for v in self.lens:
                col.append(c)
                c += round_up(v, 8)
            self._vt = (h2d(col or [0], torch.int32, self.device), c + 8)
        return self._vt


_RAGGED_1D = True


def round_up(v, m):
    return (v + m - 1) // m * m


def pack_conv_weight(w, dtype_code, c_mult=64):
    n, c, k = w.shape
    n_pad, c_pad = round_up(n, 32), round_up(c, c_mult)
    wp = torch.zeros(n_pad, c_pad, k, dtype=torch.float32, device=w.device)
    wp[:n, :c] = w.float()
    wp = wp.permute(2, 0, 1).reshape(k, n_pad // 32, 32, c_pad // 16, 2, 8)
    wp = wp.permute(0, 3, 1, 4, 2, 5).contiguous().reshape(-1)
    return wp.to(torch_dtype(dtype_code))


def pack_conv_weight_split(w, c_mult=32):
    n, c, k = w.shape
    w = w.detach().float()
    n_pad = round_up(n, 32)
    amax = w.abs().reshape(n, -1).amax(dim=1)
    e = torch.frexp(amax)[1]
    s = torch.where(amax > 0, 15 - e, torch.zeros_like(e)).clamp(-60, 60).to(torch.int32)
    scale = ((127 + s) << 23).view(torch.float32)
    ws = w * scale.view(-1, 1, 1)
    hi = ws.half()
    lo = (ws - hi.float()).half()
    ph = pack_conv_weight(hi.float(), F16, c_mult).view(-1, 8)
    pl = pack_conv_weight(lo.float(), F16, c_mult).view(-1, 8)
    inv = torch.ones(n_pad, dtype=torch.float32, device=w.device)
    inv[:n] = ((127 - s) << 23).view(torch.float32)
    return torch.stack([ph, pl], dim=1).reshape(-1).contiguous(), inv.contiguous()


def bf16x3_terms(w):
    w = w.detach().float()
    b0 = w.bfloat16()
    r1 = w - b0.float()
    b1 = r1.bfloat16()
    b2 = (r1 - b1.float()).bfloat16()
    return b0, b1, b2


def pack_conv_weight_bf16x3(w, c_mult=32):
    planes = [pack_conv_weight(t.float(), F32, c_mult).view(-1, 8).bfloat16() for t in bf16x3_terms(w)]
    return torch.stack(planes, dim=1).reshape(-1).contiguous()


def pack_unit_weight_bf16x3_k32(w):
    n_out, c_in, k = w.shape
    if n_out % 16 or c_in % 32:
        raise ValueError("pack_unit_weight_bf16x3_k32: channels must be a multiple of 32")
    planes = []
    for t in bf16x3_terms(w):
        v = t.permute(2, 1, 0).reshape(k, c_in // 32, 4, 8, n_out // 16, 16).permute(0, 1, 4, 2, 5, 3)
        planes.append(v.reshape(-1, 8))
    return torch.stack(planes, dim=1).reshape(-1).contiguous()


def pack_conv_weight_bf16x3_k32(w, c_mult=64):
    n, c, k = w.shape
    n_pad, c_pad = round_up(n, 32), round_up(c, c_mult)
    wp = torch.zeros(n_pad, c_pad, k, dtype=torch.float32, device=w.device)
    wp[:n, :c] = w.detach().float()
    return pack_unit_weight_bf16x3_k32(wp)


class PreparedWeight:
    inv, layout = None, 0

    def __init__(self, w, c_mult):
        self._src, self._c_mult, self._f32 = w.detach(), c_mult, None

    def f32(self):
        if self._f32 is None:
            self._f32 = pack_conv_weight(self._src, F32, self._c_mult)
        return self._f32


class SplitWeight(PreparedWeight):
    code = F32S

    def __init__(self, w, c_mult=64):
        super().__init__(w, c_mult)
        self.packed, self.inv = pack_conv_weight_split(w, c_mult)


class EmulWeight(PreparedWeight):

    def __init__(self, w, c_mult=64, code=F32E, layout=None):
        super().__init__(w, c_mult)
        self.code = code
        self.layout = (1 if c_mult % 64 == 0 else 0) if layout is None else layout
        self.packed = pack_conv_weight_bf16x3_k32(w, c_mult) if self.layout else pack_conv_weight_bf16x3(w, c_mult)


def conv_halo_fits(k_w, dil):
    return (k_w - 1) * dil <= 32


_OPERAND = [F32]


@contextlib.contextmanager
def operands(precision):
    rec = None if precision is None else _precision.record(precision)
    prev, _OPERAND[0] = _OPERAND[0], rec.operand if rec is not None and rec.tensors == F32 else F32
    try:
        yield
    finally:
        _OPERAND[0] = prev


def operand_code():
    return _OPERAND[0]


ATTENTION_PRECISIONS = ("fp32", "fp32_bf16x3")
ATTENTION_F32_PRECISIONS = tuple(sorted(n for n, p in _precision.TABLE.items() if p.tensors == F32))
_ATTENTION = [None]


def check_attention_precision(precision, attention):
    if precision not in PRECISIONS:
        raise ValueError(precision)
    if attention is None:
        return
    if attention not in ATTENTION_PRECISIONS:
        raise ValueError(f"attention={attention!r}: None (what the precision implies) or one of {ATTENTION_PRECISIONS}")
    if precision not in ATTENTION_F32_PRECISIONS:
        raise ValueError(f"attention={attention!r} needs f32 activations: precision one of {ATTENTION_F32_PRECISIONS}, not {precision!r}")


@contextlib.contextmanager
def attention_precision(attention):
    prev, _ATTENTION[0] = _ATTENTION[0], attention
    try:
        yield
    finally:
        _ATTENTION[0] = prev


def emul_attention_wins(n_heads, d_k, rel_mode):
    return False


def attention_dtype(dtype, split, attention, n_heads, d_k, rel_mode):
    if attention is None or dtype != F32:
        return F32S if split else dtype
    if attention == "fp32_bf16x3" and emul_attention_wins(n_heads, d_k, rel_mode):
        return F32E
    return F32


def operand(code, w, c_mult=64):
    return SplitWeight(w, c_mult) if code == F32S else EmulWeight(w, c_mult, code) if code in EMUL else pack_conv_weight(w, code, c_mult)


def f32_operand(w, c_mult=64):
    return operand(_OPERAND[0], w, c_mult)


def _pack_dev_args(w, c_mult, dgrad):
    lib = _abi.load()
    w = _dev(w)
    if w.dtype != torch.float32 or not w.is_contiguous():
        w = w.float().contiguous()
    n, c, k = w.shape
    pn, pc = (c, n) if dgrad else (n, c)
    return lib, w, (n, c, k), round_up(pn, 32), round_up(pc, c_mult)


def pack_conv_weight_dev(w, dtype_code, c_mult=64, dgrad=False):
    lib, w, (n, c, k), n_pad, c_pad = _pack_dev_args(w, c_mult, dgrad)
    out = torch.empty(k * n_pad * c_pad, dtype=torch_dtype(dtype_code), device=w.device)
    _abi.check(lib.jatts_pack_conv_weight(w.data_ptr(), n, c, k, c_mult, int(dgrad), dtype_code, out.data_ptr(), _stream()),
               "jatts_pack_conv_weight")
    return out, c_pad


def pack_conv_weight_split_dev(w, c_mult=64, dgrad=False):
    lib, w, (n, c, k), n_pad, c_pad = _pack_dev_args(w, c_mult, dgrad)
    out = torch.empty(2 * k * n_pad * c_pad, dtype=torch.float16, device=w.device)
    inv = torch.empty(n_pad, dtype=torch.float32, device=w.device)
    _abi.check(lib.jatts_pack_conv_weight_split(w.data_ptr(), n, c, k, c_mult, int(dgrad), out.data_ptr(), inv.data_ptr(), _stream()),
               "jatts_pack_conv_weight_split")
    return out, inv, c_pad


def pack_conv_weight_bf16x3_dev(w, c_mult=64, dgrad=False):
    lib, w, (n, c, k), n_pad, c_pad = _pack_dev_args(w, c_mult, dgrad)
    out = torch.empty(3 * k * n_pad * c_pad, dtype=torch.bfloat16, device=w.device)
    _abi.check(lib.jatts_pack_conv_weight_bf16x3(w.data_ptr(), n, c, k, c_mult, int(dgrad), out.data_ptr(), _stream()), "jatts_pack_conv_weight_bf16x3")
    return out, c_pad


def convtranspose_as_conv(w, stride, padding):
    c_in, c_out, K = w.shape
    qs = [(r, q) for r in range(stride) for q in range(-K, K + 1) if 0 <= stride * q + r + padding < K]
    qmin, qmax = min(q for _, q in qs), max(q for _, q in qs)
    taps = qmax - qmin + 1
    wc = torch.zeros(stride * c_out, c_in, taps, dtype=w.dtype, device=w.device)
    for r, q in qs:
        kk = stride * q + r + padding
        wc[r * c_out:(r + 1) * c_out, :, qmax - q] = w[:, :, kk].t()
    return wc, qmax


def conv1d(rb, xs, w_packed, c_in, n_out, k_w, *, dtype, dil=1, pad=None, bias=None, act=ACT_NONE,
           alpha=1.0, resid=None, out=None, out_f32=False, transposed=False, pre_lrelu=None,
           in_scale=1.0, ldx=None, x_col0=0, len_mul=1, out_ld=None, out_col0=0, out_rows=None, resid_col0=0,
           y_seq_col0=None, reflect=False, variant=0, w_inv=None, snake=None, split=None, w_layout=0):
    lib = _abi.load()
    if isinstance(xs, torch.Tensor):
        xs = [xs]
    if isinstance(w_packed, PreparedWeight):
        if dtype != F32:
            raise ValueError(f"conv1d: a {type(w_packed).__name__} goes with dtype F32 tensors")
        if conv_halo_fits(k_w, dil):
            dtype, w_inv, w_layout, w_packed, out_f32 = w_packed.code, w_packed.inv, w_packed.layout, w_packed.packed, True
        else:
            w_packed = w_packed.f32()
    x0 = _dev(xs[0])
    rows = rb.total * len_mul
    tdt = torch_dtype(dtype)
    for x in xs:
        if x.dtype != tdt or not x.is_contiguous():
            raise ValueError(f"conv1d: inputs must be contiguous {tdt}")
    ldx = ldx if ldx is not None else x0.shape[-1]
    if x0.numel() < rows * ldx or max(x_col0 if isinstance(x_col0, (list, tuple)) else [x_col0]) + c_in > ldx:
        raise ValueError("conv1d: input too small for the ragged geometry")
    if pad is None:
        pad = (k_w - 1) // 2 * dil
    n_pad = round_up(n_out, 32)
    if dtype == F32S:
        if w_packed.dtype != torch.float16 or w_packed.numel() != 2 * n_pad * c_in * k_w or w_inv is None or w_inv.numel() != n_pad:
            raise ValueError("conv1d: F32S takes the (packed, inverse scales) pair of pack_conv_weight_split")
    elif dtype in EMUL:
        if w_packed.dtype != torch.bfloat16 or w_packed.numel() != 3 * n_pad * c_in * k_w:
            raise ValueError("conv1d: F32E / F32E6 take the packed bf16 terms of pack_conv_weight_bf16x3")
        out_f32 = True
    elif w_packed.dtype != tdt or w_packed.numel() != n_pad * c_in * k_w:
        raise ValueError("conv1d: packed weight has wrong dtype/size")
    odt = torch.float32 if out_f32 else tdt
    out2 = None
    if split is not None:
        n_split, ld2, col2 = split
        if transposed or out is not None or resid is not None or n_split % 256 or not 0 < n_split < n_out:
            raise ValueError("conv1d: split takes a fresh row-major output, no residual, n_split a multiple of 256 below n_out")
        out = torch.empty(rows, out_ld or n_split, dtype=odt, device=x0.device)
        out2 = torch.empty(n_out - n_split, ld2, dtype=odt, device=x0.device)
    if out is None:
        if transposed:
            out = torch.empty(n_out, rows if out_ld is None else out_ld, dtype=odt, device=x0.device)
        else:
            out = torch.empty(rows if out_rows is None else out_rows, out_ld or n_out, dtype=odt, device=x0.device)
    if out.dtype != odt:
        raise ValueError("conv1d: output dtype mismatch")
    ldy = out.shape[-1] if out_ld is None else out_ld
    d = _abi.ConvDesc()
    d.rg = rb.struct(len_mul)
    d.dtype, d.n_in = dtype, len(xs)
    cols = x_col0 if isinstance(x_col0, (list, tuple)) else [x_col0] * len(xs)
    for i, x in enumerate(xs):
        d.x[i] = _ptr(x, cols[i])
    d.pad_mode = _abi.PAD_REFLECT if reflect else _abi.PAD_ZERO
    d.variant = variant
    d.ldx, d.in_scale = ldx, in_scale
    d.pre_act = _abi.PRE_LRELU if pre_lrelu is not None else _abi.PRE_NONE
    d.pre_slope = pre_lrelu or 0.0
    d.w, d.c_in, d.n_out, d.k_w, d.dil, d.pad = w_packed.data_ptr(), c_in, n_out, k_w, dil, pad
    d.bias = _ptr(bias)
    d.act, d.alpha = act, alpha
    if snake is not None:
        if act != ACT_NONE or any(v.dtype != torch.float32 or v.numel() != n_out or not v.is_contiguous() for v in snake):
            raise ValueError("conv1d: snake takes two contiguous f32 vectors of n_out and replaces act")
        d.act, d.act_a, d.act_b = _abi.ACT_SNAKEBETA, snake[0].data_ptr(), snake[1].data_ptr()
    if resid is not None:
        if resid.dtype != torch.float32:
            raise ValueError("conv1d: residual must be f32")
        d.resid, d.ldr = _ptr(resid, resid_col0), resid.shape[-1]
    d.y, d.ldy = _ptr(out, out_col0), ldy
    d.y_is_f32, d.y_transposed = int(odt == torch.float32), int(transposed)
    d.y_seq_col0 = _ptr(y_seq_col0) if transposed else None
    d.w_inv = _ptr(w_inv) if dtype == F32S else None
    d.w_layout = w_layout if dtype in EMUL else 0
    if out2 is not None:
        d.n_split, d.ldy2, d.y2, d.y2_seq_col0 = split[0], split[1], out2.data_ptr(), _ptr(split[2])
    _count(2.0 * c_in * n_out * k_w * rows)
    with _Timed("conv1d", (c_in, n_out, k_w, rows)):
        _abi.check(lib.jatts_conv1d(C.byref(d), _stream()), "jatts_conv1d")
    return out if out2 is None else (out, out2)


def _check_unit_weights(who, dtype, channels, k_w, *ws):
    n = channels * channels * k_w
    want = {F32: (torch.float32, n), F16: (torch.float16, n), F32S: (torch.float16, 2 * n), F32E: (torch.bfloat16, 3 * n), F32E6: (torch.bfloat16, 3 * n)}[dtype]
    for w in ws:
        if w.dtype != want[0] or w.numel() != want[1] or not w.is_cuda:
            raise ValueError(f"{who}: dtype code {dtype} needs packed weights of {want[1]} x {want[0]} on the GPU (pack_conv_weight / pack_conv_weight_split / "
                             f"pack_conv_weight_bf16x3 with c_mult=32), got {w.numel()} x {w.dtype}")


def _resunit_desc(rb, len_mul, x, y, w1, b1, w2, b2, channels, k_w, dil, slope, dtype, add, out_scale, ws, w_layout, variant):
    d = _abi.ResUnitDesc()
    d.w_layout, d.variant = w_layout, variant
    d.rg = rb.struct(len_mul)
    d.dtype, d.channels, d.k_w, d.dil, d.slope = dtype, channels, k_w, dil, slope
    rows = rb.total * len_mul
    if x.numel() != rows * channels or y.numel() != rows * channels or x.dtype != torch_dtype(dtype):
        raise ValueError("hifigan_resunit: bad buffer size/dtype")
    d.x, d.y = _dev(x).data_ptr(), y.data_ptr()
    _check_unit_weights("hifigan_resunit", dtype, channels, k_w, *((w1,) if w2 is None else (w1, w2)))
    d.w1, d.b1, d.w2, d.b2 = w1.data_ptr(), b1.data_ptr(), _ptr(w2), _ptr(b2)
    if dtype == F32S:
        need = ws[:1] if ws is not None and w2 is None else ws
        if need is None or any(v is None or v.numel() < channels or v.dtype != torch.float32 for v in need):
            raise ValueError("hifigan_resunit: F32S needs the inverse weight scales (pack_conv_weight_split)")
        d.ws1, d.ws2 = ws[0].data_ptr(), _ptr(ws[1]) if len(ws) > 1 else None
    if add:
        for a in add:
            if a.numel() != rows * channels or a.dtype != x.dtype:
                raise ValueError("hifigan_resunit: bad mix buffer")
        d.add0 = add[0].data_ptr()
        d.add1 = add[1].data_ptr() if len(add) > 1 else None
    d.out_scale = out_scale
    return d


def hifigan_resunit(rb, len_mul, x, y, w1, b1, w2, b2, channels, k_w, dil, slope, dtype, add=None, out_scale=1.0, ws=None, w_layout=0, variant=0):
    lib = _abi.load()
    d = _resunit_desc(rb, len_mul, x, y, w1, b1, w2, b2, channels, k_w, dil, slope, dtype, add, out_scale, ws, w_layout, variant)
    with _Timed("resunit", (channels, k_w, dil, rb.total * len_mul, len(add) if add else 0)):
        _abi.check(lib.jatts_hifigan_resunit(C.byref(d), _stream()), "jatts_hifigan_resunit")
    return y


def resunit_variant(rb, len_mul, x, y, w1, b1, w2, b2, channels, k_w, dil, slope, dtype, add=None, out_scale=1.0, ws=None, w_layout=0, variant=0):
    lib = _abi.load()
    d = _resunit_desc(rb, len_mul, x, y, w1, b1, w2, b2, channels, k_w, dil, slope, dtype, add, out_scale, ws, w_layout, variant)
    rc = lib.jatts_resunit_variant(C.byref(d))
    _abi.check(min(rc, 0), "jatts_resunit_variant")
    return rc


def hifigan_resblock(rb, len_mul, x, y, units, channels, k_w, slope, dtype, add=None, out_scale=1.0, ws=None):
    lib = _abi.load()
    d = _abi.ResBlockDesc()
    d.rg = rb.struct(len_mul)
    d.dtype, d.channels, d.k_w, d.n_units, d.slope = dtype, channels, k_w, len(units), slope
    rows = rb.total * len_mul
    if x.numel() != rows * channels or y.numel() != rows * channels or x.dtype != torch_dtype(dtype):
        raise ValueError("hifigan_resblock: bad buffer size/dtype")
    d.x, d.y = _dev(x).data_ptr(), y.data_ptr()
    for i, (w1, b1, w2, b2, dil) in enumerate(units):
        _check_unit_weights("hifigan_resblock", dtype, channels, k_w, w1, w2)
        d.w1[i], d.b1[i], d.w2[i], d.b2[i], d.dil[i] = w1.data_ptr(), b1.data_ptr(), w2.data_ptr(), b2.data_ptr(), dil
    if dtype == F32S:
        if ws is None or len(ws) != len(units):
            raise ValueError("hifigan_resblock: F32S needs the inverse weight scales of every unit")
        for i, (a, b) in enumerate(ws):
            d.ws1[i], d.ws2[i] = a.data_ptr(), b.data_ptr()
    if add:
        for a in add:
            if a.numel() != rows * channels or a.dtype != x.dtype:
                raise ValueError("hifigan_resblock: bad mix buffer")
        d.add0 = add[0].data_ptr()
        d.add1 = add[1].data_ptr() if len(add) > 1 else None
    d.out_scale = out_scale
    with _Timed("resblock", (channels, k_w, tuple(u[4] for u in units), rows, len(add) if add else 0)):
        _abi.check(lib.jatts_hifigan_resblock(C.byref(d), _stream()), "jatts_hifigan_resblock")
    return y


def hifigan_output(rb, len_mul, xs, in_scale, slope, c_in, k_w, w, bias, dtype):
    lib = _abi.load()
    rows = rb.total * len_mul
    y = torch.empty(rows, dtype=torch.float32, device=xs[0].device)
    arr = (C.c_void_p * len(xs))(*[_dev(x).data_ptr() for x in xs])
    rg = rb.struct(len_mul)
    _abi.check(lib.jatts_hifigan_output(C.byref(rg), dtype, arr, len(xs), in_scale, slope, c_in, k_w,
                                        w.data_ptr(), float(bias), y.data_ptr(), _stream()),
               "jatts_hifigan_output")
    return y


def relpos_attention(rb, q, ldq, k, ldk, vt, ldvt, g, ldg, ku, scale, n_heads, d_k, dtype,
                     q_col0=0, k_col0=0, rel_mode=1, rel_center=0, vt_col0=None, kv_len=None):
    lib = _abi.load()
    out = torch.empty(rb.total, n_heads * d_k, dtype=torch_dtype(dtype), device=q.device)
    d = _abi.RelAttnDesc()
    d.rg = rb.struct()
    d.dtype, d.n_heads, d.d_k = dtype, n_heads, d_k
    d.q, d.ldq = _ptr(_dev(q), q_col0), ldq
    d.k, d.ldk = _ptr(k, k_col0), ldk
    d.vt, d.ldvt = vt.data_ptr(), ldvt
    d.g, d.ldg = _ptr(g), ldg
    d.ku = _ptr(ku)
    d.scale = scale
    d.out, d.ldo = out.data_ptr(), n_heads * d_k
    d.rel_mode, d.rel_center = rel_mode, rel_center
    d.vt_col0 = _ptr(vt_col0)
    d.kv_len = _ptr(kv_len)
    with _Timed("relattn", (n_heads, d_k, rb.total, sum(v * v for v in rb.lens))):
        _abi.check(lib.jatts_relpos_attention(C.byref(d), _stream()), "jatts_relpos_attention")
    return out


def rowdot(x, ldx, rows, n_heads, d_k, vec, col0=0):
    lib = _abi.load()
    out = torch.empty(rows, n_heads, dtype=torch.float32, device=x.device)
    _abi.check(lib.jatts_rowdot(code_of(x), _ptr(_dev(x), col0), ldx, rows, n_heads, d_k, vec.data_ptr(),
                                out.data_ptr(), _stream()), "jatts_rowdot")
    return out


_BAD_IDS = {}


def _bad_counter(dev):
    key = dev.index if dev.index is not None else torch.cuda.current_device()
    t = _BAD_IDS.get(key)
    if t is None:
        t = _BAD_IDS[key] = torch.zeros(1, dtype=torch.int64, device=dev)
    return t


def embed_scale(ids, table, scale, n_bad=None):
    lib = _abi.load()
    if n_bad is None:
        n_bad = _bad_counter(_dev(ids).device)
    out = torch.empty(ids.numel(), table.shape[1], dtype=torch.float32, device=ids.device)
    _abi.check(lib.jatts_embed_scale(_dev(ids).data_ptr(), ids.numel(), table.data_ptr(), table.shape[1],
                                     float(scale), out.data_ptr(), table.shape[0], _ptr(n_bad), _stream()), "jatts_embed_scale")
    return out


def check_bad_ids(device):
    t = _BAD_IDS.get(torch.device(device).index if torch.device(device).index is not None else torch.cuda.current_device())
    if t is None:
        return
    n = int(t)
    if n:
        t.zero_()
        raise IndexError(f"index out of range in self ({n} token ids outside the embedding table)")


def bad_ids_async(device):
    dev = torch.device(device)
    t = _BAD_IDS.get(dev.index if dev.index is not None else torch.cuda.current_device())
    if t is None:
        return lambda wait=False: True
    host = torch.zeros(1, dtype=torch.int64).pin_memory()
    host.copy_(t, non_blocking=True)
    t.zero_()
    ev = torch.cuda.Event()
    ev.record()

    def resolve(wait=False):
        if wait:
            ev.synchronize()
        elif not ev.query():
            return False
        if int(host):
            n = int(host)
            host.zero_()
            raise IndexError(f"index out of range in self ({n} token ids outside the embedding table in an earlier training step)")
        return True
    return resolve


def layernorm(x, gamma, beta, out_dtype, eps=1e-12, out=None):
    lib = _abi.load()
    rows, dim = x.shape
    if out is None:
        out = torch.empty(rows, dim, dtype=torch_dtype(out_dtype), device=x.device)
    _abi.check(lib.jatts_layernorm(_dev(x).data_ptr(), code_of(x), dim, out.data_ptr(), out_dtype, dim, rows,
                                   dim, gamma.data_ptr(), beta.data_ptr(), eps, _stream()), "jatts_layernorm")
    return out


def affine_cast(x, out_dtype, scale=None, shift=None, ldy=None, x_col0=0, dim=None, out=None, out_col0=0):
    lib = _abi.load()
    rows, ldx = x.shape
    dim = dim if dim is not None else ldx - x_col0
    fresh = out is None
    if fresh:
        ldy = ldy or dim
        out = torch.empty(rows, ldy, dtype=torch_dtype(out_dtype), device=x.device)
        dim_w = dim
    else:
        ldy, dim_w = out.shape[1], dim
        if out.dtype != torch_dtype(out_dtype) or out.shape[0] != rows or out_col0 + dim > ldy:
            raise ValueError("affine_cast: bad output slice")
    fn = lib.jatts_affine_cast if fresh else lib.jatts_affine_slice
    _abi.check(fn(_ptr(_dev(x), x_col0), ldx, _ptr(out, out_col0), out_dtype, ldy, rows, dim_w,
                  _ptr(scale), _ptr(shift), _stream()), "jatts_affine_cast")
    return out


def glu_dwconv_bn_swish(rb, x, channels, k_w, w_dw, bn_scale, bn_shift, dtype):
    lib = _abi.load()
    y = torch.empty(rb.total, channels, dtype=torch_dtype(dtype), device=x.device)
    rg = rb.struct()
    _abi.check(lib.jatts_glu_dwconv_bn_swish(C.byref(rg), dtype, _dev(x).data_ptr(), y.data_ptr(), channels,
                                             k_w, w_dw.data_ptr(), bn_scale.data_ptr(), bn_shift.data_ptr(),
                                             _stream()), "jatts_glu_dwconv_bn_swish")
    return y


def predictor_head(x, w, b, want_duration=False, offset=1.0):
    lib = _abi.load()
    rows, dim = x.shape
    v = torch.empty(rows, dtype=torch.float32, device=x.device)
    dur = torch.empty(rows, dtype=torch.int64, device=x.device) if want_duration else None
    _abi.check(lib.jatts_predictor_head(code_of(x), _dev(x).data_ptr(), dim, rows, dim, w.data_ptr(), float(b),
                                        v.data_ptr(), _ptr(dur), offset, _stream()), "jatts_predictor_head")
    return (v, dur) if want_duration else v


def variance_embed_add(rb, hs, p, wp, bp, e, we, be):
    lib = _abi.load()
    rg = rb.struct()
    _abi.check(lib.jatts_variance_embed_add(C.byref(rg), _dev(hs).data_ptr(), hs.shape[1], p.data_ptr(),
                                            wp.data_ptr(), bp.data_ptr(), wp.shape[-1], e.data_ptr(),
                                            we.data_ptr(), be.data_ptr(), we.shape[-1], _stream()),
               "jatts_variance_embed_add")
    return hs


def gated_tanh_sigmoid(rb, x, gseq, channels, dtype):
    lib = _abi.load()
    y = torch.empty(rb.total, channels, dtype=torch_dtype(dtype), device=x.device)
    rg = rb.struct()
    _abi.check(lib.jatts_gated_tanh_sigmoid(C.byref(rg), dtype, _dev(x).data_ptr(), _ptr(gseq), y.data_ptr(),
                                            channels, _stream()), "jatts_gated_tanh_sigmoid")
    return y


def groupnorm_mish(rb, x, channels, groups, gamma, beta, out_dtype, eps=1e-5, addvec=None, time_split=True):
    lib = _abi.load()
    y = torch.empty(rb.total, channels, dtype=torch_dtype(out_dtype), device=x.device)
    rg = rb.struct()
    ws = None
    if time_split:
        ws = torch.empty(rb.n_seq * groups * ((rb.max_len + 63) // 64) * 3, dtype=torch.float32, device=x.device)
    _abi.check(lib.jatts_groupnorm_mish(C.byref(rg), _dev(x).data_ptr(), code_of(x), y.data_ptr(), out_dtype, channels,
                                        groups, gamma.data_ptr(), beta.data_ptr(), eps, _ptr(addvec), _ptr(ws), _stream()),
               "jatts_groupnorm_mish")
    return y


def snakebeta(x, alpha, inv_beta):
    lib = _abi.load()
    y = torch.empty_like(x)
    _abi.check(lib.jatts_snakebeta(code_of(x), _dev(x).data_ptr(), y.data_ptr(), x.shape[0], x.shape[1],
                                   alpha.data_ptr(), inv_beta.data_ptr(), _stream()), "jatts_snakebeta")
    return y


def l2_normalize(x, out_dtype, ldy=None, eps=1e-12):
    lib = _abi.load()
    rows, dim = x.shape
    ldy = ldy or dim
    y = torch.empty(rows, ldy, dtype=torch_dtype(out_dtype), device=x.device)
    _abi.check(lib.jatts_l2_normalize(_dev(x).data_ptr(), dim, y.data_ptr(), out_dtype, ldy, rows, dim, eps,
                                      _stream()), "jatts_l2_normalize")
    return y


def gaussian_sample(stats, noise, noise_scale):
    lib = _abi.load()
    rows, c2 = stats.shape
    z = torch.empty(rows, c2 // 2, dtype=torch.float32, device=stats.device)
    _abi.check(lib.jatts_gaussian_sample(_dev(stats).data_ptr(), noise.data_ptr(), z.data_ptr(), rows, c2 // 2,
                                         float(noise_scale), _stream()), "jatts_gaussian_sample")
    return z


def flip_channels(x):
    lib = _abi.load()
    y = torch.empty_like(x)
    _abi.check(lib.jatts_flip_channels(_dev(x).data_ptr(), y.data_ptr(), x.shape[0], x.shape[1], _stream()),
               "jatts_flip_channels")
    return y


def add_seq_vector(rb, hs, vec):
    lib = _abi.load()
    rg = rb.struct()
    _abi.check(lib.jatts_add_seq_vector(C.byref(rg), _dev(hs).data_ptr(), hs.shape[1], vec.data_ptr(),
                                        _stream()), "jatts_add_seq_vector")
    return hs


# ... 932 lines not shown
```

### jatts_amd/vocoder/hifigan.py

```python

import torch

from .. import hip
from ..graphs import GraphCache
from ..models._conformer import PackedConv
from ..models._prepared import Prepared
from ..models import _schema as S
from ..precision import TABLE


class UnitConv:

    def __init__(self, w, b, code, k32=False, also32=False):
        self.n_out, self.c_in, self.k = w.shape
        self.inv, self.layout = None, 1 if (k32 and code in hip.EMUL) else 0
        if code == hip.F32S:
            self.w, self.inv = hip.pack_conv_weight_split(w, 32)
        elif code in hip.EMUL:
            self.w = hip.pack_unit_weight_bf16x3_k32(w) if k32 else hip.pack_conv_weight_bf16x3(w, 32)
        else:
            self.w = hip.pack_conv_weight(w, code, 32)
        self.w_block = hip.pack_conv_weight_bf16x3(w, 32) if (self.layout and also32) else self.w
        self.b = b.detach().float().contiguous()


class HiFiGANGenerator(Prepared, torch.nn.Module):
    def __init__(self, in_channels=80, out_channels=1, channels=512, kernel_size=7,
                 upsample_scales=(8, 8, 2, 2), upsample_kernel_sizes=(16, 16, 4, 4),
                 resblock_kernel_sizes=(3, 7, 11), resblock_dilations=((1, 3, 5), (1, 3, 5), (1, 3, 5)),
                 use_additional_convs=True, bias=True, nonlinear_activation="LeakyReLU",
                 nonlinear_activation_params=None, use_weight_norm=True, **unused):
        super().__init__()
        if nonlinear_activation != "LeakyReLU":
            raise NotImplementedError("only LeakyReLU generators are supported")
        if out_channels != 1:
            raise NotImplementedError("out_channels must be 1")
        self.use_additional_convs, self.bias = bool(use_additional_convs), bool(bias)
        if len(upsample_scales) != len(upsample_kernel_sizes):
            raise ValueError("upsample_scales / upsample_kernel_sizes mismatch")
        self.slope = float((nonlinear_activation_params or {"negative_slope": 0.1}).get("negative_slope", 0.1))
        self.in_channels, self.channels, self.kernel_size = in_channels, channels, kernel_size
        self.upsample_scales = tuple(int(s) for s in upsample_scales)
        self.upsample_kernel_sizes = tuple(int(k) for k in upsample_kernel_sizes)
        self.resblock_kernel_sizes = tuple(int(k) for k in resblock_kernel_sizes)
        self.resblock_dilations = tuple(tuple(int(d) for d in ds) for ds in resblock_dilations)
        if channels % (1 << len(self.upsample_scales)) or channels > 512:
            raise NotImplementedError("channels must be divisible by 2**n_upsamples and <= 512")
        for s_, uk in zip(self.upsample_scales, self.upsample_kernel_sizes):
            if uk != 2 * s_:
                raise NotImplementedError(f"upsample_kernel_size {uk} != 2 * scale {s_}: only the k = 2s geometry of the HiFi-GAN recipes is supported")
        if not 1 <= len(self.resblock_kernel_sizes) <= 3:
            raise NotImplementedError("1..3 ResBlocks per stage (the MRF mix kernels take up to 3 inputs)")
        self.hop = 1
        for s in self.upsample_scales:
            self.hop *= s
        spec = S.new_spec()
        S._conv(spec, "input_conv", channels, in_channels, kernel_size)
        nb = len(self.resblock_kernel_sizes)
        c = channels
        for i, uk in enumerate(self.upsample_kernel_sizes):
            spec[f"upsamples.{i}.1.weight"] = ((c, c // 2, uk), "param")
            if self.bias:
                spec[f"upsamples.{i}.1.bias"] = ((c // 2,), "param")
            c //= 2
            for j, rk in enumerate(self.resblock_kernel_sizes):
                for d in range(len(self.resblock_dilations[j])):
                    S._conv(spec, f"blocks.{i * nb + j}.convs1.{d}.1", c, c, rk, bias=self.bias)
                    if self.use_additional_convs:
                        S._conv(spec, f"blocks.{i * nb + j}.convs2.{d}.1", c, c, rk, bias=self.bias)
        S._conv(spec, "output_conv.1", out_channels, c, kernel_size)
        S.build_from_spec(self, spec)
        self.eval()

    def load_state_dict(self, state_dict, strict=True, **kw):
        sd = {}
        for k, v in state_dict.items():
            if k.endswith("weight_g"):
                stem = k[:-len("weight_g")]
                wv = state_dict[stem + "weight_v"]
                norm = wv.reshape(wv.shape[0], -1).norm(dim=1).reshape(-1, *([1] * (wv.dim() - 1)))
                sd[stem + "weight"] = v * wv / norm
            elif k.endswith("weight_v") or k in ("mean", "scale"):
                continue
            else:
                sd[k] = v
        return super().load_state_dict(sd, strict=strict, **kw)

    def remove_weight_norm(self):
        return None

    def set_precision(self, precision):
        if precision == "fp32_split" and not self.use_additional_convs:
            raise NotImplementedError("fp32_split (JATTS_F32S) has no single-conv dilation unit: generators with use_additional_convs=False run in "
                                      "fp32, fp16, fp32_bf16x3 or fp32_bf16x3_6p")
        return super().set_precision(precision)

    HAS_ATTENTION = False
    GPU_ONLY = "jatts_amd HiFiGANGenerator runs on the GPU only (no CPU fallback)"

    def _prep_device(self):
        return self.input_conv.weight.device

    def _prepare_packed(self, dev, key, dt):
        udt = TABLE[self.precision].operand
        sd = self.state_dict()
        f32 = lambda t: t.detach().float().to(dev).contiguous()
        fset, fhalo = {hip.F16: (self.fused_blocks, 64), hip.F32: (self.fused_blocks_f32, 16), hip.F32S: (self.fused_blocks_split, 64)}.get(
            udt, (self.fused_blocks_emul, 64))
        P = {"key": key, "dtype": dt, "dev": dev, "unit_dtype": udt, "fused_blocks": fset, "fused_halo": fhalo}
        nb = len(self.resblock_kernel_sizes)
        P["ups"], P["blocks"] = [], []
        supported = {hip.F16: (32, 64, 128, 256, 512), hip.F32: (32, 64, 128, 256)}[dt]
        P["unit_channels"] = supported

        def cp(c):
            for v in supported:
                if c <= v:
                    return v
            raise NotImplementedError(f"{c} channels exceed the widest fused-unit tile for this precision")

        def padw(w, n, c):
            w = w.detach().float()
            o = torch.zeros(n, c, w.shape[2], dtype=torch.float32)
            o[: w.shape[0], : w.shape[1]] = w
            return o

        def padb(b, n):
            o = torch.zeros(n, dtype=torch.float32)
            if b is not None:
                o[: b.numel()] = b.detach().float()
            return o

        c_prev = hip.round_up(self.channels, 64)
        P["in"] = PackedConv(padw(sd["input_conv.weight"], c_prev, sd["input_conv.weight"].shape[1]), padb(sd["input_conv.bias"], c_prev), dt, dev)
        for i, (s, uk) in enumerate(zip(self.upsample_scales, self.upsample_kernel_sizes)):
            w = sd[f"upsamples.{i}.1.weight"].detach().float()
            c_out = cp(w.shape[1])
            if i + 1 < len(self.upsample_scales):
                c_out = max(c_out, 64)
            wp = torch.zeros(c_prev, c_out, w.shape[2], dtype=torch.float32)
            wp[: w.shape[0], : w.shape[1]] = w
            wc, pad = hip.convtranspose_as_conv(wp, s, s // 2 + s % 2)
            pc = PackedConv(wc, padb(sd.get(f"upsamples.{i}.1.bias"), c_out).repeat(s), dt, dev)
            P["ups"].append((pc, pad, s, c_out))
            stage = []
            for j, rk in enumerate(self.resblock_kernel_sizes):
                units = []
                for di, d in enumerate(self.resblock_dilations[j]):
                    q = f"blocks.{i * nb + j}."
                    k32 = c_out % 32 == 0
                    also32 = self.use_additional_convs and (c_out, rk) in self.fused_blocks_emul
                    mk = lambda w, b: UnitConv(w, b, udt, k32, also32)
                    c1 = mk(padw(sd[q + f"convs1.{di}.1.weight"], c_out, c_out).to(dev), padb(sd.get(q + f"convs1.{di}.1.bias"), c_out).to(dev))
                    c2 = mk(padw(sd[q + f"convs2.{di}.1.weight"], c_out, c_out).to(dev), padb(sd.get(q + f"convs2.{di}.1.bias"), c_out).to(dev)) \
                        if self.use_additional_convs else None
                    units.append((c1, c2, rk, d))
                stage.append(units)
            P["blocks"].append(stage)
            c_prev = c_out
        wo = padw(sd["output_conv.1.weight"], 1, c_prev)
        P["out_w"] = f32(wo[0].t())
        P["out_b"] = float(sd["output_conv.1.bias"].detach().float()[0])
        self._prep = P
        return P

    fused_blocks = frozenset({(32, 3), (32, 7), (64, 3)})
    fused_blocks_f32 = frozenset({(32, 3)})
    fused_blocks_split = frozenset({(32, 3), (32, 7), (64, 3)})

    fused_blocks_emul = frozenset({(32, 3)})

    @torch.no_grad()
    def inference_batch(self, rb, mel, scale=None, shift=None, taps=None):
        P = self._prepare()
        if rb.n_seq == 1 and taps is None:
            gc = P.get("graphs")
            if gc is None:
                gc = P["graphs"] = GraphCache()
            affine = tuple(t for t in (scale, shift) if t is not None)

            def body(mel_, *aff):
                it = iter(aff)
                return self._generate(P, hip.RaggedBatch(rb.lens, rb.device), mel_, next(it) if scale is not None else None,
                                      next(it) if shift is not None else None, None)
            return gc.run(("generate", rb.total, scale is not None, shift is not None), body, (mel,) + affine)
        return self._generate(P, rb, mel, scale, shift, taps)

    def _generate(self, P, rb, mel, scale, shift, taps):
        dt, udt = P["dtype"], P["unit_dtype"]
        pin = P["in"]
        x = hip.affine_cast(mel, dt, scale=scale, shift=shift, ldy=pin.c_in)
        x = hip.conv1d(rb, x, pin.w, pin.c_in, pin.n_out, pin.k, dtype=dt, bias=pin.b)
        if taps is not None:
            taps["input_conv"] = x.float()
        xs, in_scale, rate = [x], 1.0, 1
        supported = P["unit_channels"]
        for i, (pc, pad, s, c_out) in enumerate(P["ups"]):
            rows = rb.total * rate
            up = hip.conv1d(rb, xs, pc.w, pc.c_in, pc.n_out, pc.k, dtype=dt, bias=pc.b, pad=pad,
                            pre_lrelu=self.slope, in_scale=in_scale, len_mul=rate)
            rate *= s
            up = up.view(rows * s, c_out)
            if taps is not None:
                taps[f"up{i}"] = up.float()
            outs = []
            blocks = P["blocks"][i]
            fuse_mean = c_out in supported and len(blocks) in (2, 3)
            bufs = [[torch.empty_like(up), torch.empty_like(up)] for _ in blocks]
            for j, units in enumerate(blocks):
                cur = up
                if self.use_additional_convs and (c_out, units[0][2]) in P["fused_blocks"] and len(units) <= 3 \
                        and sum((units[0][2] - 1) // 2 * (u[3] + 1) for u in units) <= P["fused_halo"]:
                    lastb = fuse_mean and j == len(blocks) - 1
                    hip.hifigan_resblock(rb, rate, cur, bufs[j][0], [(c1.w_block, c1.b, c2.w_block, c2.b, d) for c1, c2, _, d in units],
                                         c_out, units[0][2], self.slope, udt, add=outs if lastb else None,
                                         out_scale=1.0 / len(blocks) if lastb else 1.0,
                                         ws=[(c1.inv, c2.inv) for c1, c2, _, _ in units] if udt == hip.F32S else None)
                    outs.append(bufs[j][0])
                    continue
                for di, (c1, c2, rk, d) in enumerate(units):
                    nxt = bufs[j][di & 1]
                    last = fuse_mean and j == len(blocks) - 1 and di == len(units) - 1
                    hip.hifigan_resunit(rb, rate, cur, nxt, c1.w, c1.b, c2.w if c2 else None, c2.b if c2 else None, c_out, rk, d, self.slope, udt,
                                        add=outs if last else None, out_scale=1.0 / len(blocks) if last else 1.0,
                                        ws=(c1.inv, c2.inv) if udt == hip.F32S else None, w_layout=c1.layout)
                    cur = nxt
                outs.append(cur)
            if fuse_mean:
                xs, in_scale = [outs[-1]], 1.0
            else:
                xs, in_scale = outs, 1.0 / len(outs)
            if taps is not None:
                taps[f"mrf{i}"] = sum(o.float() for o in xs) * in_scale
        return hip.hifigan_output(rb, rate, xs, in_scale, 0.01, xs[0].shape[1], self.kernel_size,
                                  P["out_w"], P["out_b"], dt)

    @torch.no_grad()
    def inference(self, c, normalize_before=False):
        if normalize_before:
            raise NotImplementedError("normalize_before=True needs registered stats; jatts passes False (vocoder.py:64)")
        if not isinstance(c, torch.Tensor):
            c = torch.tensor(c, dtype=torch.float)
        dev = self.input_conv.weight.device
        c = c.to(dev).float().contiguous()
        rb = hip.RaggedBatch([c.shape[0]], dev)
        return self.inference_batch(rb, c).view(-1, 1)
```

Before: 70.03 million samples/s.

## Skip structurally zero taps in polyphase transposed-conv upsampling

Transposed-conv upsamplers are lowered to a polyphase conv whose packed weight is zero outside a per-phase tap window. This adds a per-output-group tap table so the direct f32 and emulated conv kernels only iterate over the nonzero taps of each group, shifting weight and activation offsets by the window start. It is meant to remove wasted MFMA work and weight loads on the HiFi-GAN upsampling layers. The cost is added plumbing, host-side validation that the weights really are zero outside the windows, and extra kernel instantiations.

```diff
diff --git a/include/jatts_hip.h b/include/jatts_hip.h
--- a/include/jatts_hip.h
+++ b/include/jatts_hip.h
@@ -84,6 +84,10 @@
 } jatts_conv_desc;
 
 int jatts_conv1d(const jatts_conv_desc* d, void* stream);
+
+int jatts_conv1d_taps(const jatts_conv_desc* d, int32_t group_channels, int32_t taps_per_group, const int32_t* tap_first, void* stream);
+
+int64_t jatts_conv1d_taps_ksteps(const jatts_conv_desc* d, int32_t group_channels, int32_t taps_per_group, const int32_t* tap_first);
 
 int64_t jatts_conv_weight_index(int32_t n, int32_t tap, int32_t c, int32_t n_pad, int32_t c_in);
 
diff --git a/jatts_amd/_abi.py b/jatts_amd/_abi.py
--- a/jatts_amd/_abi.py
+++ b/jatts_amd/_abi.py
@@ -65,6 +65,8 @@
     "jatts_last_error": (C.c_char_p, []),
     "jatts_device_info": (C.c_int, [C.c_char_p, C.c_int]),
     "jatts_conv1d": (C.c_int, [C.POINTER(ConvDesc), C.c_void_p]),
+    "jatts_conv1d_taps": (C.c_int, [C.POINTER(ConvDesc), C.c_int32, C.c_int32, C.POINTER(C.c_int32), C.c_void_p]),
+    "jatts_conv1d_taps_ksteps": (C.c_int64, [C.POINTER(ConvDesc), C.c_int32, C.c_int32, C.POINTER(C.c_int32)]),
     "jatts_conv_weight_index": (C.c_int64, [C.c_int32] * 5),
     "jatts_hifigan_resunit": (C.c_int, [C.POINTER(ResUnitDesc), C.c_void_p]),
     "jatts_resunit_variant": (C.c_int, [C.POINTER(ResUnitDesc)]),
diff --git a/jatts_amd/csrc/conv1d_direct.h b/jatts_amd/csrc/conv1d_direct.h
--- a/jatts_amd/csrc/conv1d_direct.h
+++ b/jatts_amd/csrc/conv1d_direct.h
@@ -1,6 +1,7 @@
 #pragma once
 #include "conv1d_impl.h"
 #include "unit_frame.h"
+#include "conv_taps.h"
 
 namespace {
 
@@ -24,8 +25,9 @@
 #undef JATTS_ACT_LOOP
 }
 
-template <int NF, int NT, int WN, int WT, int D, int DIAG = 0, bool PRE = false, bool SNAKE = false>
-__global__ __launch_bounds__(WN* WT * 64, (D <= 2 ? 3 : 2)) void conv1d_direct_kernel(jatts_conv_desc d, unsigned long long* trace, unsigned trace_cap, XcdOrder xo) {
+template <int NF, int NT, int WN, int WT, int D, int DIAG = 0, bool PRE = false, bool SNAKE = false, bool TAPS = false>
+__global__ __launch_bounds__(WN* WT * 64, (D <= 2 ? 3 : 2)) void conv1d_direct_kernel(jatts_conv_desc d, unsigned long long* trace, unsigned trace_cap, XcdOrder xo,
+                                                                                  ConvTaps tp) {
   int bx, by, bz;
   if (!xo.decode(blockIdx.x, bx, by, bz, d.rg, WT * NT * 32)) return;
   JATTS_TRACE_BEGIN(trace, trace_cap, blockIdx.x);
@@ -67,18 +69,24 @@
 #pragma unroll
   for (int t = 0; t < NT; ++t) vx[t] = (unsigned)(((t0 + col0 + t * 32 + (lane & 31) - d.pad) * d.ldx + 8 * g) * 4);
   const unsigned tap_stride = (unsigned)(d.dil * d.ldx * 4);
+  int tap0 = 0, k_eff = d.k_w;
+  if constexpr (TAPS) {
+    conv_taps_window(tp, nf0 * 32, (nf0 + NF) * 32, d.n_out, d.k_w, tap0, k_eff);
+    tap0 = __builtin_amdgcn_readfirstlane(tap0);
+    k_eff = __builtin_amdgcn_readfirstlane(k_eff);
+  }
   int p_kc = 0, p_tap = 0;
-  const int last_kc = KC16 - 1, last_tap = d.k_w - 1;
+  const int last_kc = KC16 - 1, last_tap = k_eff - 1;
   auto ldb8 = [](const __amdgpu_buffer_rsrc_t& r, unsigned voff, unsigned soff) {
     const f32x4 lo = __builtin_bit_cast(f32x4, __builtin_amdgcn_raw_buffer_load_b128(r, voff, soff, 0));
     const f32x4 hi = __builtin_bit_cast(f32x4, __builtin_amdgcn_raw_buffer_load_b128(r, voff + 16, soff, 0));
     return f32x8{lo[0], lo[1], lo[2], lo[3], hi[0], hi[1], hi[2], hi[3]};
   };
   auto issue = [&](f32x8(&a)[NF], f32x8(&bq)[NT]) {
-    const unsigned sw = (unsigned)((p_tap * KC16 + p_kc) * NFR) << 11;
+    const unsigned sw = (unsigned)(((tap0 + p_tap) * KC16 + p_kc) * NFR) << 11;
 #pragma unroll
     for (int f = 0; f < NF; ++f) a[f] = ldb8(rw, vw[f], sw);
-    const unsigned shift = (unsigned)p_tap * tap_stride, sx = (unsigned)p_kc << 6;
+    const unsigned shift = (unsigned)(tap0 + p_tap) * tap_stride, sx = (unsigned)p_kc << 6;
 #pragma unroll
     for (int t = 0; t < NT; ++t) bq[t] = ldb8(rx, vx[t] + shift, sx);
     ++p_tap;
@@ -89,7 +97,7 @@
 #pragma unroll
   for (int j = 0; j < D; ++j) issue(ra[j], rb[j]);
   __builtin_amdgcn_sched_barrier(0);
-  const int n_steps = KC16 * d.k_w;
+  const int n_steps = KC16 * k_eff;
   JATTS_STAMP(2);
   for (int s0 = 0; s0 < n_steps; s0 += D) {
 #pragma unroll
@@ -161,15 +169,22 @@
          (maxL + 256 + (int64_t)d.k_w * d.dil) * ld * 4 < (int64_t)1 << 31 && (int64_t)d.k_w * d.c_in * n_pad * 4 < (int64_t)1 << 31;
 }
 
-template <int NF, int NT, int WN, int WT, int D, int DIAG = 0, bool PRE = false, bool SNAKE = false>
-int launch_conv_direct(const jatts_conv_desc& d, hipStream_t s) {
+inline int conv_direct_tile(const jatts_conv_desc& d) {
+  const int64_t maxL = (int64_t)d.rg.max_len * d.rg.len_mul;
+  const int64_t t128 = (maxL + 127) / 128, t64 = (maxL + 63) / 64;
+  const int64_t wgs = t128 * d.rg.n_seq * ((d.n_out + 127) / 128);
+  return (wgs <= 512 || t64 * 64 * 23 <= t128 * 128 * 20) ? 5 : 3;
+}
+
+template <int NF, int NT, int WN, int WT, int D, int DIAG = 0, bool PRE = false, bool SNAKE = false, bool TAPS = false>
+int launch_conv_direct(const jatts_conv_desc& d, hipStream_t s, const ConvTaps& tp = ConvTaps()) {
   constexpr int BT = WT * NT * 32, BN = WN * NF * 32;
   const int64_t maxL = (int64_t)d.rg.max_len * d.rg.len_mul;
   XcdOrder xo;
   const int64_t total = xo.plan((int)((maxL + BT - 1) / BT), d.rg.n_seq, (d.n_out + BN - 1) / BN, (int64_t)BN * d.c_in * d.k_w * 4, ragged_tiles_1d(d.rg, BT));
   if (total >= (int64_t)1 << 31) return jatts_set_error_msg(JATTS_ERR_UNSUPPORTED, "conv1d: launch too large");
-  hipLaunchKernelGGL((conv1d_direct_kernel<NF, NT, WN, WT, D, DIAG, PRE, SNAKE>), dim3((unsigned)total), dim3(WN * WT * 64), 0, s, d, jatts_g_trace,
-                     jatts_g_trace_cap, xo);
+  hipLaunchKernelGGL((conv1d_direct_kernel<NF, NT, WN, WT, D, DIAG, PRE, SNAKE, TAPS>), dim3((unsigned)total), dim3(WN * WT * 64), 0, s, d, jatts_g_trace,
+                     jatts_g_trace_cap, xo, tp);
   JATTS_CHECK_LAUNCH();
   return JATTS_OK;
 }
diff --git a/jatts_amd/csrc/conv1d_emul.hip b/jatts_amd/csrc/conv1d_emul.hip
--- a/jatts_amd/csrc/conv1d_emul.hip
+++ b/jatts_amd/csrc/conv1d_emul.hip
@@ -1,4 +1,4 @@
-#include "conv1d_emul16.h"
+#include "conv1d_emul16_tiles.h"
 
 template <typename T>
 static int conv1d_emul(const jatts_conv_desc& d, hipStream_t s) {
@@ -15,22 +15,6 @@
   else return launch_conv_emul<T, 2, 2, 2, 2, 1, 32, 2>(d, s);
 }
 
-template <typename T>
-static int conv1d_emul16(const jatts_conv_desc& d, hipStream_t s) {
-  const int variant = d.variant;
-  if (d.n_in > 1) return launch_conv_emul16<T, 4, 4, 2, 2, 3, 64, 1>(d, s);
-  if (d.n_out <= 64) return launch_conv_emul16<T, 2, 2, 2, 2, 1, 64, 2>(d, s);
-  const int64_t maxL = (int64_t)d.rg.max_len * d.rg.len_mul;
-  const int64_t t64 = ((maxL + 63) / 64) * d.rg.n_seq;
-  const int64_t wgs128 = ((maxL + 127) / 128) * d.rg.n_seq * ((d.n_out + 127) / 128);
-  const bool ok384 = d.n_split % 384 == 0;
-  if (ok384 && (variant == 6 || (variant == 0 && d.n_out % 384 == 0 && t64 * (d.n_out / 384) >= 256))) return launch_conv_emul16<T, 3, 4, 8, 1, 1, 64, 1, 32, 1>(d, s);
-  if (variant == 3 || (variant == 0 && d.n_out % 256 == 0 && t64 * (d.n_out / 256) >= 256)) return launch_conv_emul16<T, 2, 4, 8, 1, 1, 64, 1>(d, s);
-  if (variant == 9 || (variant == 0 && t64 * ((d.n_out + 127) / 128) <= 256)) return launch_conv_emul16<T, 2, 2, 4, 1, 1, 64, 2>(d, s);
-  if (variant == 1 || (variant == 0 && (d.k_w == 1 || wgs128 <= 128))) return launch_conv_emul16<T, 2, 4, 4, 1, 1, 64, 2>(d, s);
-  return launch_conv_emul16<T, 2, 4, 4, 2, 1, 64, 1>(d, s);
-}
-
 int jatts_conv1d_emul(const jatts_conv_desc& d, hipStream_t s) {
   if (d.w_layout == 1) return d.dtype == JATTS_F32E6 ? conv1d_emul16<bf3f>(d, s) : conv1d_emul16<bf3>(d, s);
   return d.dtype == JATTS_F32E6 ? conv1d_emul<bf3f>(d, s) : conv1d_emul<bf3>(d, s);
diff --git a/jatts_amd/csrc/conv1d_emul16.h b/jatts_amd/csrc/conv1d_emul16.h
--- a/jatts_amd/csrc/conv1d_emul16.h
+++ b/jatts_amd/csrc/conv1d_emul16.h
@@ -2,6 +2,7 @@
 #include "conv1d_emul.h"
 #include "unit_frame.h"
 #include "resunit_emul16_impl.h"
+#include "conv_taps.h"
 
 #ifndef JATTS_CEMUL_ANTIPHASE
 #define JATTS_CEMUL_ANTIPHASE 1
@@ -26,8 +27,8 @@
   int KC32, NFR16, k_w, kc_per, n_chunks;
   int p_chunk, p_tap, p_kk;
 
-  __device__ __forceinline__ void init(const T* w, int KC32_, int NFR16_, int nf0, int k_w_, int kc_per_, int n_chunks_, int lane) {
-    wbase = w + (size_t)lane * 8;
+  __device__ __forceinline__ void init(const T* w, int KC32_, int NFR16_, int nf0, int k_w_, int kc_per_, int n_chunks_, int lane, int tap0 = 0) {
+    wbase = w + (size_t)lane * 8 + ((size_t)tap0 * KC32_ * NFR16_) * 512;
     KC32 = KC32_; NFR16 = NFR16_; k_w = k_w_; kc_per = kc_per_; n_chunks = n_chunks_;
 #pragma unroll
     for (int f = 0; f < NF; ++f) nfo[f] = (nf0 + f < NFR16 ? nf0 + f : NFR16 - 1) * 512;
@@ -58,11 +59,11 @@
 
 template <typename T, int NF, int NT, int D>
 __device__ __forceinline__ void conv_stage16(typename Acc16<T>::type (&acc)[NF][NT], WRing16<T, NF, D>& ring, int kc_per, int k_w, int dil, const char* act,
-                                             int pitch, int col0, int lane) {
+                                             int pitch, int col0, int lane, int row0 = 0) {
   typedef typename Elem<T>::vec8 V8;
   static_assert(NT % 2 == 0, "column fragments come in pairs");
   const int n_it = k_w * kc_per;
-  const char* bbase = act + (size_t)(col0 + (lane & 15)) * pitch + (size_t)(lane >> 4) * 48;
+  const char* bbase = act + (size_t)(row0 + col0 + (lane & 15)) * pitch + (size_t)(lane >> 4) * 48;
   const int last_tap = k_w - 1;
   int bp_tap = 0, bp_kk = 0;
   auto next_b = [&]() {
@@ -194,8 +195,8 @@
   }
 }
 
-template <typename T, int NF, int NT, int WN, int WT, int NIN, int KCHT, int OCC, int HALO = 32, int D = 2>
-__global__ __launch_bounds__(WN* WT * 64, OCC) void conv1d_emul16_kernel(jatts_conv_desc d, int f32_tile, XcdOrder xo JATTS_CEMUL_TRACE_PARAMS) {
+template <typename T, int NF, int NT, int WN, int WT, int NIN, int KCHT, int OCC, int HALO = 32, int D = 2, bool TAPS = false>
+__global__ __launch_bounds__(WN* WT * 64, OCC) void conv1d_emul16_kernel(jatts_conv_desc d, int f32_tile, XcdOrder xo, ConvTaps tp JATTS_CEMUL_TRACE_PARAMS) {
   extern __shared__ __attribute__((aligned(16))) char smem[];
   constexpr int BT = WT * NT * 16, NTHR = WN * WT * 64, BN = WN * NF * 16;
   int bx, b, bz;
@@ -253,7 +254,13 @@
   static_assert((KCHT / 32) % D == 0 || D % (KCHT / 32) == 0, "ring depth and steps per chunk and tap");
   WRing16<T, NF, D> ring;
   const int n_chunks = d.c_in / KCHT;
-  ring.init((const T*)d.w, KC32, NFR16, nf0, d.k_w, KCHT / 32, n_chunks, lane);
+  int tap0 = 0, k_eff = d.k_w;
+  if constexpr (TAPS) {
+    conv_taps_window(tp, nf0 * 16, (nf0 + NF) * 16, d.n_out, d.k_w, tap0, k_eff);
+    tap0 = __builtin_amdgcn_readfirstlane(tap0);
+    k_eff = __builtin_amdgcn_readfirstlane(k_eff);
+  }
+  ring.init((const T*)d.w, KC32, NFR16, nf0, k_eff, KCHT / 32, n_chunks, lane, tap0);
   const size_t buf_bytes = (size_t)rows * pitch;
   StageRegs<float, MAXU, NIN> sr;
   int64_t soff[MAXU];
@@ -297,7 +304,7 @@
       if (ci + 2 < n_chunks) issue((ci + 2) * KCHT);
     } else if (more && !(JATTS_CEMUL_DIAG & 2)) issue((ci + 1) * KCHT);
     JATTS_PH(1);
-    conv_stage16<T, NF, NT, D>(accx, ring, KCHT / 32, d.k_w, d.dil, smem + (size_t)(ci & 1) * buf_bytes, pitch, col0, lane);
+    conv_stage16<T, NF, NT, D>(accx, ring, KCHT / 32, k_eff, d.dil, smem + (size_t)(ci & 1) * buf_bytes, pitch, col0, lane, tap0 * d.dil);
     JATTS_PH(2);
 #if JATTS_CEMUL_TRACE
     asm volatile("s_waitcnt vmcnt(0)" ::: "memory");
@@ -365,13 +372,26 @@
   trace_out();
 }
 
-template <typename T, int NF, int NT, int WN, int WT, int NIN, int KCHT, int OCC, int HALO = 32, int D = 2>
-int launch_conv_emul16(const jatts_conv_desc& d, hipStream_t s) {
+template <typename T, int NF, int NT, int WN, int WT, int NIN, int KCHT, int OCC, int HALO = 32, int D = 2, bool TAPS = false>
+int launch_conv_emul16(const jatts_conv_desc& d, hipStream_t s, const ConvTaps& tp = ConvTaps(), int64_t* ksteps = nullptr) {
   constexpr int BT = WT * NT * 16, BN = WN * NF * 16;
+  static_assert(!TAPS || (KCHT / 32) % D == 0, "tap windows: the ring depth must divide the K-steps of ONE tap");
   if ((d.k_w - 1) * d.dil > HALO) return jatts_set_error_msg(JATTS_ERR_UNSUPPORTED, "conv1d (emulated): halo beyond the staging registers");
   if (d.c_in % KCHT) return jatts_set_error_msg(JATTS_ERR_UNSUPPORTED, "conv1d (emulated): c_in must be a multiple of the chunk width");
   const int64_t maxL = (int64_t)d.rg.max_len * d.rg.len_mul;
   dim3 grid((unsigned)((maxL + BT - 1) / BT), (unsigned)d.rg.n_seq, (unsigned)((d.n_out + BN - 1) / BN));
+  if (ksteps) {
+    int64_t n = 0;
+    for (int bz = 0; bz < (int)grid.z; ++bz)
+      for (int wn = 0; wn < WN; ++wn) {
+        const int nf0 = (bz * WN + wn) * NF;
+        int tap0, k_eff;
+        conv_taps_window(tp, nf0 * 16, (nf0 + NF) * 16, d.n_out, d.k_w, tap0, k_eff);
+        n += (int64_t)WT * (d.c_in / KCHT) * k_eff * (KCHT / 32);
+      }
+    *ksteps = n;
+    return JATTS_OK;
+  }
   const size_t rows = (size_t)BT + (size_t)(d.k_w - 1) * d.dil;
   size_t lds = 2 * rows * (KCHT * 6 + 16);
   int f32_tile = 0;
@@ -380,15 +400,15 @@
     f32_tile = 1;
     if (lds < (size_t)BT * (BN * 4 + 16)) lds = (size_t)BT * (BN * 4 + 16);
   }
-  constexpr auto kern = conv1d_emul16_kernel<T, NF, NT, WN, WT, NIN, KCHT, OCC, HALO, D>;
+  constexpr auto kern = conv1d_emul16_kernel<T, NF, NT, WN, WT, NIN, KCHT, OCC, HALO, D, TAPS>;
   if (const int rc = unit_lds_ready<kern>(JATTS_SITE("conv1d (emulated): tile exceeds 160 KiB LDS"), lds)) return rc;
   XcdOrder xo;
   const int64_t total = xo.plan((int)grid.x, (int)grid.y, (int)grid.z, (int64_t)BN * d.c_in * d.k_w * 6, ragged_tiles_1d(d.rg, BT));
   if (total >= (int64_t)1 << 31) return jatts_set_error_msg(JATTS_ERR_UNSUPPORTED, "conv1d: launch too large");
 #if JATTS_CEMUL_TRACE
-  hipLaunchKernelGGL(kern, dim3((unsigned)total), dim3(WN * WT * 64), lds, s, d, f32_tile, xo, jatts_g_trace, jatts_g_trace_cap);
+  hipLaunchKernelGGL(kern, dim3((unsigned)total), dim3(WN * WT * 64), lds, s, d, f32_tile, xo, tp, jatts_g_trace, jatts_g_trace_cap);
 #else
-  hipLaunchKernelGGL(kern, dim3((unsigned)total), dim3(WN * WT * 64), lds, s, d, f32_tile, xo);
+  hipLaunchKernelGGL(kern, dim3((unsigned)total), dim3(WN * WT * 64), lds, s, d, f32_tile, xo, tp);
 #endif
   JATTS_CHECK_LAUNCH();
   return JATTS_OK;
diff --git a/jatts_amd/csrc/conv1d_emul16_tiles.h b/jatts_amd/csrc/conv1d_emul16_tiles.h
--- /dev/null
+++ b/jatts_amd/csrc/conv1d_emul16_tiles.h
@@ -0,0 +1,18 @@
+#pragma once
+#include "conv1d_emul16.h"
+
+template <typename T, bool TAPS = false>
+static int conv1d_emul16(const jatts_conv_desc& d, hipStream_t s, const ConvTaps& tp = ConvTaps(), int64_t* ksteps = nullptr) {
+  const int variant = d.variant;
+  if (d.n_in > 1) return launch_conv_emul16<T, 4, 4, 2, 2, 3, 64, 1, 32, 2, TAPS>(d, s, tp, ksteps);
+  if (d.n_out <= 64) return launch_conv_emul16<T, 2, 2, 2, 2, 1, 64, 2, 32, 2, TAPS>(d, s, tp, ksteps);
+  const int64_t maxL = (int64_t)d.rg.max_len * d.rg.len_mul;
+  const int64_t t64 = ((maxL + 63) / 64) * d.rg.n_seq;
+  const int64_t wgs128 = ((maxL + 127) / 128) * d.rg.n_seq * ((d.n_out + 127) / 128);
+  const bool ok384 = d.n_split % 384 == 0;
+  if (ok384 && (variant == 6 || (variant == 0 && d.n_out % 384 == 0 && t64 * (d.n_out / 384) >= 256))) return launch_conv_emul16<T, 3, 4, 8, 1, 1, 64, 1, 32, 1, TAPS>(d, s, tp, ksteps);
+  if (variant == 3 || (variant == 0 && d.n_out % 256 == 0 && t64 * (d.n_out / 256) >= 256)) return launch_conv_emul16<T, 2, 4, 8, 1, 1, 64, 1, 32, 2, TAPS>(d, s, tp, ksteps);
+  if (variant == 9 || (variant == 0 && t64 * ((d.n_out + 127) / 128) <= 256)) return launch_conv_emul16<T, 2, 2, 4, 1, 1, 64, 2, 32, 2, TAPS>(d, s, tp, ksteps);
+  if (variant == 1 || (variant == 0 && (d.k_w == 1 || wgs128 <= 128))) return launch_conv_emul16<T, 2, 4, 4, 1, 1, 64, 2, 32, 2, TAPS>(d, s, tp, ksteps);
+  return launch_conv_emul16<T, 2, 4, 4, 2, 1, 64, 1, 32, 2, TAPS>(d, s, tp, ksteps);
+}
diff --git a/jatts_amd/csrc/conv1d_emul_taps.hip b/jatts_amd/csrc/conv1d_emul_taps.hip
--- /dev/null
+++ b/jatts_amd/csrc/conv1d_emul_taps.hip
@@ -0,0 +1,5 @@
+#include "conv1d_emul16_tiles.h"
+
+int jatts_conv1d_emul_taps(const jatts_conv_desc& d, hipStream_t s, const ConvTaps& tp, int64_t* ksteps) {
+  return d.dtype == JATTS_F32E6 ? conv1d_emul16<bf3f, true>(d, s, tp, ksteps) : conv1d_emul16<bf3, true>(d, s, tp, ksteps);
+}
diff --git a/jatts_amd/csrc/conv1d_f32_direct.hip b/jatts_amd/csrc/conv1d_f32_direct.hip
--- a/jatts_amd/csrc/conv1d_f32_direct.hip
+++ b/jatts_amd/csrc/conv1d_f32_direct.hip
@@ -8,12 +8,7 @@
     if (variant != 0 && variant != 3) return 1;
     return d.pre_act != JATTS_PRE_NONE ? launch_conv_direct<2, 2, 1, 4, 2, 0, true>(d, s) : launch_conv_direct<2, 2, 1, 4, 2>(d, s);
   }
-  if (variant == 0) {
-    const int64_t maxL = (int64_t)d.rg.max_len * d.rg.len_mul;
-    const int64_t t128 = (maxL + 127) / 128, t64 = (maxL + 63) / 64;
-    const int64_t wgs = t128 * d.rg.n_seq * ((d.n_out + 127) / 128);
-    variant = (wgs <= 512 || t64 * 64 * 23 <= t128 * 128 * 20) ? 5 : 3;
-  }
+  if (variant == 0) variant = conv_direct_tile(d);
   if (d.pre_act != JATTS_PRE_NONE) {
     if (variant == 5) return launch_conv_direct<2, 1, 2, 2, 2, 0, true>(d, s);
     return launch_conv_direct<2, 2, 2, 2, 2, 0, true>(d, s);
diff --git a/jatts_amd/csrc/conv1d_f32_direct_taps.hip b/jatts_amd/csrc/conv1d_f32_direct_taps.hip
--- /dev/null
+++ b/jatts_amd/csrc/conv1d_f32_direct_taps.hip
@@ -0,0 +1,11 @@
+#include "conv1d_direct.h"
+
+int jatts_conv1d_f32_direct_taps(const jatts_conv_desc& d, hipStream_t s, const ConvTaps& tp) {
+  int variant = d.variant;
+  if (variant == 1 || variant == 2) return 1;
+  if (!conv_direct_ok(d) || d.pre_act != JATTS_PRE_LRELU || d.act == JATTS_ACT_SNAKEBETA || d.n_out <= 64) return 1;
+  if (variant == 0) variant = conv_direct_tile(d);
+  if (variant == 5) return launch_conv_direct<2, 1, 2, 2, 2, 0, true, false, true>(d, s, tp);
+  if (variant == 3) return launch_conv_direct<2, 2, 2, 2, 2, 0, true, false, true>(d, s, tp);
+  return 1;
+}
diff --git a/jatts_amd/csrc/conv_api.hip b/jatts_amd/csrc/conv_api.hip
--- a/jatts_amd/csrc/conv_api.hip
+++ b/jatts_amd/csrc/conv_api.hip
@@ -1,14 +1,17 @@
 #include <stdlib.h>
 
 #include "common.h"
+#include "conv_taps.h"
 
 unsigned long long* jatts_g_trace = nullptr;
 unsigned jatts_g_trace_cap = 0;
 
 int jatts_conv1d_f16(const jatts_conv_desc& d, hipStream_t s);
 int jatts_conv1d_f32(const jatts_conv_desc& d, hipStream_t s);
+int jatts_conv1d_f32_direct_taps(const jatts_conv_desc& d, hipStream_t s, const ConvTaps& tp);
 int jatts_conv1d_split(const jatts_conv_desc& d, hipStream_t s);
 int jatts_conv1d_emul(const jatts_conv_desc& d, hipStream_t s);
+int jatts_conv1d_emul_taps(const jatts_conv_desc& d, hipStream_t s, const ConvTaps& tp, int64_t* ksteps);
 int jatts_resunit_f16_narrow(const jatts_resunit_desc& d, hipStream_t s);
 int jatts_resunit_f16_wide(const jatts_resunit_desc& d, hipStream_t s);
 int jatts_resunit_f32(const jatts_resunit_desc& d, hipStream_t s);
@@ -42,7 +45,7 @@
   return ((((int64_t)tap * KC32 + kc) * NFR16 + nf) * 64 + lane) * 8 + (c % 8);
 }
 
-extern "C" int jatts_conv1d(const jatts_conv_desc* d, void* stream) {
+static int conv1d_check(const jatts_conv_desc* d) {
   if (!d || !d->x[0] || !d->w || !d->y || !d->rg.cu_rows) return jatts_set_error_msg(JATTS_ERR_ARG, "conv1d: null pointer");
   if (d->c_in <= 0 || d->c_in % 64) return jatts_set_error_msg(JATTS_ERR_ARG, "conv1d: c_in must be a positive multiple of 64");
   if (d->ldx % 8) return jatts_set_error_msg(JATTS_ERR_ARG, "conv1d: ldx must be a multiple of 8");
@@ -55,10 +58,19 @@
   if (d->n_split != 0 && (d->n_split < 0 || d->n_split % 256 || d->n_split >= d->n_out || !d->y2 || d->y_transposed || d->resid || d->ldy2 <= 0))
     return jatts_set_error_msg(JATTS_ERR_ARG, "conv1d: n_split must be a multiple of 256 below n_out, with y2 / ldy2 set, y row-major and no residual");
   if (d->w_layout != 0 && d->dtype != JATTS_F32E && d->dtype != JATTS_F32E6) return jatts_set_error_msg(JATTS_ERR_ARG, "conv1d: w_layout = 1 goes with JATTS_F32E / JATTS_F32E6 only");
+  return JATTS_OK;
+}
+
+static int conv1d_run(const jatts_conv_desc* d, hipStream_t s, const ConvTaps* tp) {
   if (d->rg.max_len <= 0) return JATTS_OK;
-  hipStream_t s = (hipStream_t)stream;
   if (d->dtype == JATTS_F16) return jatts_conv1d_f16(*d, s);
-  if (d->dtype == JATTS_F32) return jatts_conv1d_f32(*d, s);
+  if (d->dtype == JATTS_F32) {
+    if (tp) {
+      const int rc = jatts_conv1d_f32_direct_taps(*d, s, *tp);
+      if (rc != 1) return rc;
+    }
+    return jatts_conv1d_f32(*d, s);
+  }
   if (d->dtype == JATTS_F32S) {
     if (!d->w_inv) return jatts_set_error_msg(JATTS_ERR_ARG, "conv1d: JATTS_F32S needs w_inv");
     if (!d->y_is_f32) return jatts_set_error_msg(JATTS_ERR_ARG, "conv1d: JATTS_F32S writes f32 (y_is_f32 = 1)");
@@ -67,9 +79,50 @@
   if (d->dtype == JATTS_F32E || d->dtype == JATTS_F32E6) {
     if (!d->y_is_f32) return jatts_set_error_msg(JATTS_ERR_ARG, "conv1d: JATTS_F32E / JATTS_F32E6 write f32 (y_is_f32 = 1)");
     if (d->w_layout != 0 && d->w_layout != 1) return jatts_set_error_msg(JATTS_ERR_ARG, "conv1d: w_layout must be 0 or 1");
-    return jatts_conv1d_emul(*d, s);
+    return tp ? jatts_conv1d_emul_taps(*d, s, *tp, nullptr) : jatts_conv1d_emul(*d, s);
   }
   return jatts_set_error_msg(JATTS_ERR_ARG, "conv1d: unknown dtype");
+}
+
+extern "C" int jatts_conv1d(const jatts_conv_desc* d, void* stream) {
+  if (const int rc = conv1d_check(d)) return rc;
+  return conv1d_run(d, (hipStream_t)stream, nullptr);
+}
+
+static int conv1d_taps_table(const jatts_conv_desc* d, int32_t group_channels, int32_t taps_per_group, const int32_t* tap_first, ConvTaps* tp) {
+  if (group_channels < 1 || taps_per_group < 1 || !tap_first) return jatts_set_error_msg(JATTS_ERR_ARG, "conv1d_taps: group_channels >= 1, taps_per_group >= 1 and a table required");
+  const int64_t n_groups = ((int64_t)d->n_out + group_channels - 1) / group_channels;
+  for (int64_t g = 0; g < n_groups; ++g)
+    if (tap_first[g] < 0 || (int64_t)tap_first[g] + taps_per_group > d->k_w)
+      return jatts_set_error_msg(JATTS_ERR_ARG, "conv1d_taps: every window [tap_first[g], tap_first[g] + taps_per_group) must lie inside [0, k_w)");
+  const bool emul16 = (d->dtype == JATTS_F32E || d->dtype == JATTS_F32E6) && d->w_layout == 1;
+  if (n_groups > JATTS_CONV_TAPS_MAX_GROUPS || !(emul16 || d->dtype == JATTS_F32)) return 1;
+  tp->group_channels = group_channels;
+  tp->taps_per_group = taps_per_group;
+  tp->n_groups = (int)n_groups;
+  for (int g = 0; g < JATTS_CONV_TAPS_MAX_GROUPS; ++g) tp->tap_first[g] = (signed char)(g < n_groups ? tap_first[g] : 0);
+  return 0;
+}
+
+extern "C" int jatts_conv1d_taps(const jatts_conv_desc* d, int32_t group_channels, int32_t taps_per_group, const int32_t* tap_first, void* stream) {
+  if (const int rc = conv1d_check(d)) return rc;
+  ConvTaps tp = {};
+  const int fw = conv1d_taps_table(d, group_channels, taps_per_group, tap_first, &tp);
+  if (fw < 0) return fw;
+  return conv1d_run(d, (hipStream_t)stream, fw ? nullptr : &tp);
+}
+
+extern "C" int64_t jatts_conv1d_taps_ksteps(const jatts_conv_desc* d, int32_t group_channels, int32_t taps_per_group, const int32_t* tap_first) {
+  if (const int rc = conv1d_check(d)) return rc;
+  ConvTaps tp = {};
+  const int fw = conv1d_taps_table(d, group_channels, taps_per_group, tap_first, &tp);
+  if (fw < 0) return fw;
+  if ((d->dtype != JATTS_F32E && d->dtype != JATTS_F32E6) || d->w_layout != 1)
+    return jatts_set_error_msg(JATTS_ERR_UNSUPPORTED, "conv1d_taps_ksteps: reports the w_layout = 1 emulated conv only (every other launch forwards to jatts_conv1d)");
+  if (fw) tp = ConvTaps();
+  int64_t n = 0;
+  if (const int rc = jatts_conv1d_emul_taps(*d, nullptr, tp, &n)) return rc;
+  return n;
 }
 
 static int resunit_check(const jatts_resunit_desc* d) {
diff --git a/jatts_amd/csrc/conv_taps.h b/jatts_amd/csrc/conv_taps.h
--- /dev/null
+++ b/jatts_amd/csrc/conv_taps.h
@@ -0,0 +1,27 @@
+#pragma once
+#include <hip/hip_runtime.h>
+
+#define JATTS_CONV_TAPS_MAX_GROUPS 16
+
+struct ConvTaps {
+  int group_channels, taps_per_group, n_groups;
+  signed char tap_first[JATTS_CONV_TAPS_MAX_GROUPS];
+};
+
+__host__ __device__ inline void conv_taps_window(const ConvTaps& tp, int n_lo, int n_hi, int n_out, int k_w, int& tap0, int& k_eff) {
+  tap0 = 0;
+  k_eff = k_w;
+  if (tp.n_groups <= 0) return;
+  const int hi = (n_hi < n_out ? n_hi : n_out) - 1;
+  const int lo = n_lo < hi ? n_lo : hi;
+  const int g_lo = lo / tp.group_channels, g_hi = hi / tp.group_channels;
+  int first = k_w, end = 0;
+  for (int g = 0; g < JATTS_CONV_TAPS_MAX_GROUPS; ++g)
+    if (g >= g_lo && g <= g_hi) {
+      const int t = tp.tap_first[g];
+      first = t < first ? t : first;
+      end = t + tp.taps_per_group > end ? t + tp.taps_per_group : end;
+    }
+  tap0 = first;
+  k_eff = end - first;
+}
diff --git a/jatts_amd/hip.py b/jatts_amd/hip.py
--- a/jatts_amd/hip.py
+++ b/jatts_amd/hip.py
@@ -497,7 +497,7 @@
     return out, c_pad
 
 
-def convtranspose_as_conv(w, stride, padding):
+def convtranspose_as_conv(w, stride, padding, tap_table=False):
     c_in, c_out, K = w.shape
     qs = [(r, q) for r in range(stride) for q in range(-K, K + 1) if 0 <= stride * q + r + padding < K]
     qmin, qmax = min(q for _, q in qs), max(q for _, q in qs)
@@ -506,13 +506,29 @@
     for r, q in qs:
         kk = stride * q + r + padding
         wc[r * c_out:(r + 1) * c_out, :, qmax - q] = w[:, :, kk].t()
-    return wc, qmax
+    if not tap_table:
+        return wc, qmax
+    per = max(sum(1 for r_, _ in qs if r_ == r) for r in range(stride))
+    first = [min(min(qmax - q for r_, q in qs if r_ == r), taps - per) for r in range(stride)]
+    tap_groups = (c_out, per, first)
+    check_tap_groups(wc, tap_groups)
+    return wc, qmax, tap_groups
+
+
+def check_tap_groups(w, tap_groups):
+    group_channels, per, first = tap_groups
+    n_out, _, k = w.shape
+    assert group_channels >= 1 and per >= 1 and len(first) == -(-n_out // group_channels), "tap table does not match the weight"
+    for g, f in enumerate(first):
+        assert 0 <= f and f + per <= k, "tap window outside the weight's taps"
+        rows = w[g * group_channels:(g + 1) * group_channels]
+        assert not bool(rows[:, :, :f].any()) and not bool(rows[:, :, f + per:].any()), "conv weight is not zero outside its tap windows"
 
 
 def conv1d(rb, xs, w_packed, c_in, n_out, k_w, *, dtype, dil=1, pad=None, bias=None, act=ACT_NONE,
            alpha=1.0, resid=None, out=None, out_f32=False, transposed=False, pre_lrelu=None,
            in_scale=1.0, ldx=None, x_col0=0, len_mul=1, out_ld=None, out_col0=0, out_rows=None, resid_col0=0,
-           y_seq_col0=None, reflect=False, variant=0, w_inv=None, snake=None, split=None, w_layout=0):
+           y_seq_col0=None, reflect=False, variant=0, w_inv=None, snake=None, split=None, w_layout=0, tap_groups=None):
     lib = _abi.load()
     if isinstance(xs, torch.Tensor):
         xs = [xs]
@@ -589,10 +605,38 @@
     d.w_layout = w_layout if dtype in EMUL else 0
     if out2 is not None:
         d.n_split, d.ldy2, d.y2, d.y2_seq_col0 = split[0], split[1], out2.data_ptr(), _ptr(split[2])
+    if tap_groups is not None:
+        group_channels, taps_per_group, tap_first = tap_groups
+        if len(tap_first) != -(-n_out // group_channels):
+            raise ValueError("conv1d: tap_groups needs one first tap per group of group_channels output channels")
+        _count(2.0 * c_in * n_out * taps_per_group * rows)
+        with _Timed("conv1d", (c_in, n_out, taps_per_group, rows)):
+            _abi.check(lib.jatts_conv1d_taps(C.byref(d), group_channels, taps_per_group, (C.c_int32 * len(tap_first))(*tap_first), _stream()),
+                       "jatts_conv1d_taps")
+        return out if out2 is None else (out, out2)
     _count(2.0 * c_in * n_out * k_w * rows)
     with _Timed("conv1d", (c_in, n_out, k_w, rows)):
         _abi.check(lib.jatts_conv1d(C.byref(d), _stream()), "jatts_conv1d")
     return out if out2 is None else (out, out2)
+
+
+def conv1d_taps_ksteps(lens, c_in, n_out, k_w, dtype, tap_groups, len_mul=1, n_in=1, dil=1, variant=0):
+    lib = _abi.load()
+    d = _abi.ConvDesc()
+    stub = C.addressof(_KSTEPS_STUB)
+    d.rg = _abi.Ragged(stub, len(lens), max(lens), len_mul, 0, None)
+    d.dtype, d.n_in, d.ldx, d.in_scale, d.alpha = dtype, n_in, c_in, 1.0, 1.0
+    for i in range(n_in):
+        d.x[i] = stub
+    d.w, d.y, d.ldy, d.y_is_f32 = stub, stub, n_out, 1
+    d.c_in, d.n_out, d.k_w, d.dil, d.pad, d.variant, d.w_layout = c_in, n_out, k_w, dil, 0, variant, 1
+    group_channels, taps_per_group, tap_first = tap_groups if tap_groups is not None else (n_out, k_w, [0])
+    rc = lib.jatts_conv1d_taps_ksteps(C.byref(d), group_channels, taps_per_group, (C.c_int32 * len(tap_first))(*tap_first))
+    _abi.check(min(rc, 0), "jatts_conv1d_taps_ksteps")
+    return rc
+
+
+_KSTEPS_STUB = (C.c_int32 * 4)()
 
 
 def _check_unit_weights(who, dtype, channels, k_w, *ws):
diff --git a/jatts_amd/vocoder/hifigan.py b/jatts_amd/vocoder/hifigan.py
--- a/jatts_amd/vocoder/hifigan.py
+++ b/jatts_amd/vocoder/hifigan.py
@@ -140,9 +140,9 @@
                 c_out = max(c_out, 64)
             wp = torch.zeros(c_prev, c_out, w.shape[2], dtype=torch.float32)
             wp[: w.shape[0], : w.shape[1]] = w
-            wc, pad = hip.convtranspose_as_conv(wp, s, s // 2 + s % 2)
+            wc, pad, tg = hip.convtranspose_as_conv(wp, s, s // 2 + s % 2, tap_table=True)
             pc = PackedConv(wc, padb(sd.get(f"upsamples.{i}.1.bias"), c_out).repeat(s), dt, dev)
-            P["ups"].append((pc, pad, s, c_out))
+            P["ups"].append((pc, pad, s, c_out, tg))
             stage = []
             for j, rk in enumerate(self.resblock_kernel_sizes):
                 units = []
@@ -195,10 +195,10 @@
             taps["input_conv"] = x.float()
         xs, in_scale, rate = [x], 1.0, 1
         supported = P["unit_channels"]
-        for i, (pc, pad, s, c_out) in enumerate(P["ups"]):
+        for i, (pc, pad, s, c_out, tg) in enumerate(P["ups"]):
             rows = rb.total * rate
             up = hip.conv1d(rb, xs, pc.w, pc.c_in, pc.n_out, pc.k, dtype=dt, bias=pc.b, pad=pad,
-                            pre_lrelu=self.slope, in_scale=in_scale, len_mul=rate)
+                            pre_lrelu=self.slope, in_scale=in_scale, len_mul=rate, tap_groups=tg)
             rate *= s
             up = up.view(rows * s, c_out)
             if taps is not None:
```

Measured after the change: 70.64 million samples/s, median of 6. About the same (+0.9%).
